# Kotstantinovskiy/SonicDiffusionBayesLab

Measured on AMD Instinct MI355X. Metric: 512x512 images/sec at 50 DDIM steps, higher is better.
Workload: dtype bf16; 1 GPU; SD-1.5 512x512 DDIM 50 steps, CFG 7.5, batch=8/GPU (BASELINE configs[1]); global_batch=8, sample_size=64, parallelism=batch-shard x1, weights=SD-1.5-shaped synthetic seed 1234

## Files before the change

### include/sd_hip.h

```cpp
#ifndef SD_HIP_H
#define SD_HIP_H

#ifdef __cplusplus
extern "C" {
#endif

typedef struct sd_unet sd_unet;

typedef struct sd_unet_config {
    int sample_size;
    int in_channels;
    int out_channels;
    int num_levels;
    int block_out_channels[8];
    int layers_per_block;
    int attn_levels[8];
    int cross_attention_dim;
    int num_heads;
    int norm_num_groups;
    float norm_eps;
    int context_len;
    int weight_dtype;
    float fp8_act_scale_norm;
    float fp8_act_scale_ff;
// ... 64 lines not shown
} sd_clip_config;
typedef struct sd_unet sd_clip;
int sd_clip_create(const sd_clip_config* cfg, sd_clip** out);
int sd_clip_encode(sd_clip* c, void* stream, const int* input_ids, int batch, float* hidden_out, void* workspace,
                   long long workspace_bytes);

typedef struct sd_clip_vision_config {
    int hidden_size;
    int num_layers;
    int num_heads;
    int intermediate_size;
    int image_size;
    int patch_size;
    int projection_dim;
    float layer_norm_eps;
} sd_clip_vision_config;
typedef struct sd_unet sd_clip_vision;
int sd_clip_create_projected(const sd_clip_config* cfg, int projection_dim, int eos_token_id, sd_clip** out);
long long sd_clip_text_embeds_workspace_bytes(sd_clip* c, int batch);
int sd_clip_text_embeds(sd_clip* c, void* stream, const int* input_ids, int batch, float* text_embeds, void* workspace,
                        long long workspace_bytes);
int sd_clip_vision_create(const sd_clip_vision_config* cfg, sd_clip_vision** out);
long long sd_clip_vision_workspace_bytes(sd_clip_vision* v, int batch, int height, int width);
int sd_clip_vision_encode(sd_clip_vision* v, void* stream, const unsigned char* images, int batch, int height, int width,
                          float* image_embeds, void* workspace, long long workspace_bytes);
int sd_clip_score(void* stream, const float* image_embeds, const float* text_embeds, int batch, int dim, float* raw,
                  float* score);
int sd_clip_resize_taps(int in_size, int out_size, int first, int count, int* xmin, int* xcnt, int* coeffs);

typedef struct sd_inception sd_inception;
int sd_inception_create(sd_inception** out);
void sd_inception_destroy(sd_inception* h);
int sd_inception_num_convs(const sd_inception* h);
int sd_inception_conv_info(const sd_inception* h, int index, char* name, int name_cap, long long shape[4]);
int sd_inception_load_conv(sd_inception* h, const char* name, const float* weight_oihw, long long weight_numel,
                           const float* bias, int cout);
int sd_inception_finalize(sd_inception* h);
long long sd_inception_workspace_bytes(sd_inception* h, int batch, int tap);
int sd_inception_features(sd_inception* h, void* stream, const unsigned char* images, int batch, int height, int width,
                          int tap, float* features, void* workspace, long long workspace_bytes);
int sd_fid_accumulate(void* stream, const float* features, int batch, int dim, double* sum, double* cov_sum,
                      long long* count);
int sd_op_inception_conv(void* stream, const void* X, const void* W, const float* bias, void* Y, int B, int Hin, int Win,
                         int Cin, int Cout, int kh, int kw, int stride, int pad_h, int pad_w, int ldy, int coff, int relu);
int sd_op_maxpool3x3(void* stream, const void* X, void* Y, int B, int H, int W, int C, int stride, int pad, int ldy, int coff);
int sd_op_avgpool3x3(void* stream, const void* X, void* Y, int B, int H, int W, int C, int ldy, int coff);
int sd_op_global_mean(void* stream, const void* X, float* out, int B, int HW, int C);
int sd_op_inception_resize(void* stream, const unsigned char* images, int B, int H, int W, void* out, int out_fp32);

#define SD_PROFILE_KINDS 32
int sd_unet_forward_profiled(sd_unet* u, void* stream, const float* latents, int latent_batch, int unet_batch,
                             float timestep, float* eps_out, void* workspace, long long workspace_bytes, int cache_mode,
                             int cache_branch_id, double kind_ms[SD_PROFILE_KINDS], long long kind_launches[SD_PROFILE_KINDS],
                             double kind_flops[SD_PROFILE_KINDS], double kind_bytes[SD_PROFILE_KINDS]);

long long sd_unet_forward_op_times(sd_unet* u, void* stream, const float* latents, int latent_batch, int unet_batch,
                                   float timestep, float* eps_out, void* workspace, long long workspace_bytes, int cache_mode,
                                   int cache_branch_id, char* text, long long cap);

int sd_unet_debug_tensor(sd_unet* u, void* stream, const char* name, float* host_out, long long numel,
                         void* workspace, int unet_batch, int cache_branch_id);

int sd_sched_step(void* stream, const float* eps, int cfg, float guidance, const float* x, const float* m1,
                  const float* m2, const float* m3, const float* noise, float* prev, float* y2, float* m_out,
                  const float coef[10], long long n);

int sd_cfg_rescale_factors(void* stream, const float* eps, int batch, long long n_per_sample, float guidance,
                           float rescale, float* k_out);
int sd_sched_step_rescaled(void* stream, const float* eps, int cfg, float guidance, const float* x, const float* m1,
                           const float* m2, const float* m3, const float* noise, float* prev, float* y2, float* m_out,
                           const float coef[10], long long n, const float* k, long long n_per_sample);

int sd_op_gemm(void* stream, const void* X, long long ldx, const void* X2, long long ldx2, int K1, const void* W,
               const float* bias, const float* bias2, const void* R, long long ldr, void* C, long long ldc, int M,
               int N, int K, int epi);
int sd_op_gemm_batched(void* stream, const void* X, long long ldx, const void* W, long long w_batch_stride,
                       int rows_per_batch, const float* bias, const void* R, long long ldr, void* C, long long ldc,
                       int M, int N, int K, int epi, int sm_valid);
int sd_op_gemm_batched_softmax_ln(void* stream, const void* X, long long ldx, const void* W, long long w_batch_stride,
                                  int rows_per_batch, void* C, long long ldc, int M, int N, int K, int sm_valid,
                                  const float* rowstats, int parts, const float* c1, const float* c2, float eps);
int sd_op_conv3x3(void* stream, const void* X, const void* W, const float* bias, const float* bias2, const void* R,
                  void* Y, int B, int Hin, int Win, int Cin, int Cout, int stride, int upsample);
int sd_op_conv3x3_down_asym(void* stream, const void* X, const void* W, const float* bias, void* Y, int B, int Hin, int Win,
                            int Cin, int Cout);
int sd_op_conv3x3_kernel(int M, int N, int Cin, int Hin, int Win, int stride, int upsample, int dtype);
int sd_op_softmax_rows(void* stream, void* S, long long rows, int cols, float scale);
int sd_op_conv3x3_upsample_subpixel(void* stream, const void* X, const void* W4, const float* bias, void* Y, int B, int Hin,
                                    int Win, int Cin, int Cout);
int sd_op_conv3x3_upsample_subpixel_groupnorm(void* stream, const void* X, const void* W4, const float* bias, void* Y, int B,
                                              int Hin, int Win, int Cin, int Cout, const float* gamma, const float* beta,
                                              void* Yn, int groups, float eps, int silu);
int sd_op_groupnorm(void* stream, const void* x1, int C1, const void* x2, int C2, const float* gamma,
                    const float* beta, void* y, int B, int HW, int groups, float eps, int silu);
int sd_op_conv3x3_groupnorm(void* stream, const void* X, const void* W, const float* bias, const float* bias2,
                            const void* R, void* Y, int B, int Hin, int Win, int Cin, int Cout, const float* gamma,
                            const float* beta, void* Yn, int groups, float eps, int silu);
int sd_op_conv3x3_splitk(int M, int Cout, int Cin, int Hin, int Win, int stride, int upsample);
int sd_op_layernorm(void* stream, const void* x, const float* gamma, const float* beta, void* y, int rows, int C,
                    float eps);
int sd_op_attention(void* stream, const void* Q, long long ldq, const void* K, long long ldk, const void* V,
                    long long ldv, void* O, long long ldo, int B, int heads, int Nq, int Nk, int D, float scale);
int sd_op_gemm_qkv_headmajor(void* stream, const void* X, long long ldx, const void* W, void* Q, void* KV, int M, int C,
                             int tokens, int K);
int sd_op_attention_headmajor(void* stream, const void* Q, long long ldq, const void* K, const void* V, void* O,
                              long long ldo, int B, int heads, int Nq, int Nk, int D, float scale);
int sd_op_clip_attention(void* stream, const void* qkv, void* out, int B, int L, int H, int heads);
int sd_op_vit_attention(void* stream, const void* qkv, void* out, int B, int L, int H, int heads);
int sd_op_clip_preprocess(void* stream, const unsigned char* images, int B, int H, int W, int S, int P, unsigned char* crop,
                          void* patches);
int sd_op_conv_in(void* stream, const float* x, int Bsrc, const float* Wt, const float* bias, void* y, int B, int H,
                  int W, int Cin, int Cout);
int sd_op_conv_out(void* stream, const void* x, const void* Wp, const float* bias, float* y, int B, int H, int W,
                   int Cin, int Cout);
int sd_op_time_embedding(void* stream, float t, const void* W1, const float* b1, const void* W2, const float* b2,
                         float* scratch, float* temb, int dim_in, int dim);
int sd_op_timestep_cond(void* stream, float t, const float* cond, const void* Wc, float* row, float* emb, int cond_dim,
                        int dim);

int sd_op_ln_partials(int kind, int M, int N);
int sd_op_gemm_rowstats(void* stream, const void* X, long long ldx, const void* W, const float* bias, const void* R,
                        long long ldr, void* C, long long ldc, int M, int N, int K, float* rowstats);
int sd_op_gemm_ln(void* stream, const void* X, long long ldx, const void* Wg, const float* c1, const float* c2,
                  const float* rowstats, int parts, float eps, void* C, long long ldc, int M, int N, int K, int epi);
int sd_op_gemm_plan(void* stream, const void* X, long long ldx, const void* X2, long long ldx2, int K1, const void* W,
                    const float* bias, const float* bias2, const void* R, long long ldr, void* C, long long ldc, int M, int N,
                    int K, float* rowstats, float* stats, const float* ln_rs, int ln_parts, const float* ln_c1, float ln_eps,
                    void* KV, int hm_tokens);
int sd_op_xattn_fused_rowstats(void* stream, const void* X, const void* R, void* Y, const void* At, const void* Bw,
                               const float* bias, int M, int C, int rows_per_sample, int L, float* rowstats);
int sd_op_xattn_fused(void* stream, const void* X, const void* R, void* Y, const void* At, const void* Bw,
                      const float* bias, int M, int C, int rows_per_sample, int L);
int sd_op_xattn_fused_ln(void* stream, const void* X, const void* R, void* Y, const void* At, const void* Bw,
                         const float* bias, int M, int C, int rows_per_sample, int L, const float* ln_rowstats, int ln_parts,
                         long long ln_rows, const float* c2, float eps, float* rowstats);
int sd_op_conv3x3_ablate(void* stream, const void* X, const void* W, void* Y, int B, int Hin, int Win, int Cin, int Cout,
                         int ablate);
int sd_op_xattn_fused_stamps(void* stream, const void* X, const void* R, void* Y, const void* At, const void* Bw,
                             const float* bias, int M, int C, int rows_per_sample, int L, unsigned long long* stamps);

int sd_op_gemm_fp8(void* stream, const void* X, long long ldx, const void* W, const float* wscale, float xscale,
                   const float* bias, const void* R, long long ldr, void* C, long long ldc, int M, int N, int K, int epi,
                   int out_fp8, float oscale);
int sd_op_conv3x3_fp8(void* stream, const void* X, const void* W, const float* wscale, float xscale, const float* bias,
                      const float* bias2, const void* R, void* Y, int B, int Hin, int Win, int Cin, int Cout, int stride,
                      int upsample);
int sd_op_groupnorm_fp8(void* stream, const void* x1, int C1, const void* x2, int C2, const float* gamma,
                        const float* beta, void* y, int B, int HW, int groups, float eps, int silu, int Cpad, float oscale);
int sd_op_layernorm_fp8(void* stream, const void* x, const float* gamma, const float* beta, void* y, int rows, int C,
                        int Cpad, float eps, float oscale);
int sd_op_quantize_fp8(void* stream, const void* x_bf16, void* y_fp8, long long rows, int C, int Cpad, float scale);

#ifdef __cplusplus
}
#endif
#endif
```

### sonicdiffusionbayeslab_amd/_lib.py

```python
from __future__ import annotations

import ctypes as C
import os
import re
from typing import Optional

HERE = os.path.dirname(os.path.abspath(__file__))
LIB_PATH = os.environ.get("SD_AMD_LIB", os.path.join(HERE, "lib", "libsdhip.so"))
HEADER_PATH = os.path.normpath(os.path.join(HERE, "..", "include", "sd_hip.h"))

ABLATE_LIB_PATH = os.path.join(HERE, "lib", "libsdhip_ablate.so")

_lib: Optional[C.CDLL] = None
_ablate: Optional[C.CDLL] = None


class SdUnetConfig(C.Structure):
    _fields_ = [
        ("sample_size", C.c_int), ("in_channels", C.c_int), ("out_channels", C.c_int),
        ("num_levels", C.c_int), ("block_out_channels", C.c_int * 8), ("layers_per_block", C.c_int),
        ("attn_levels", C.c_int * 8), ("cross_attention_dim", C.c_int), ("num_heads", C.c_int),
        ("norm_num_groups", C.c_int), ("norm_eps", C.c_float), ("context_len", C.c_int),
        ("weight_dtype", C.c_int), ("fp8_act_scale_norm", C.c_float), ("fp8_act_scale_ff", C.c_float),
        ("time_cond_proj_dim", C.c_int),
# ... 13 lines not shown

class SdClipVisionConfig(C.Structure):
    _fields_ = [
        ("hidden_size", C.c_int), ("num_layers", C.c_int), ("num_heads", C.c_int), ("intermediate_size", C.c_int),
        ("image_size", C.c_int), ("patch_size", C.c_int), ("projection_dim", C.c_int), ("layer_norm_eps", C.c_float),
    ]


class SdHipError(RuntimeError):
    pass


def declared_symbols() -> list:
    src = open(HEADER_PATH).read()
    src = re.sub(r"/\*.*?\*/", "", src, flags=re.S)
    return sorted(set(re.findall(r"\b(sd_[a-z0-9_]+)\s*\(", src)))


_vp, _i, _ll, _f = C.c_void_p, C.c_int, C.c_longlong, C.c_float
_SIGS = {
    "sd_last_error": (C.c_char_p, []),
    "sd_abi_version": (_i, []),
    "sd_unet_create": (_i, [C.POINTER(SdUnetConfig), C.POINTER(_vp)]),
    "sd_unet_destroy": (None, [_vp]),
    "sd_unet_num_params": (_i, [_vp]),
    "sd_unet_param_info": (_i, [_vp, _i, C.c_char_p, _i, C.POINTER(_ll), C.POINTER(_i)]),
    "sd_unet_load_param": (_i, [_vp, C.c_char_p, _vp, _ll]),
    "sd_unet_finalize": (_i, [_vp]),
    "sd_unet_debug_packed": (_ll, [_vp, C.c_char_p, _vp, _ll]),
    "sd_unet_calibrate_fp8": (_i, [_vp, _vp, _vp, _i, _i, _f, _f, _vp, _ll]),
    "sd_unet_fp8_scale_count": (_i, [_vp]),
    "sd_unet_fp8_scale_info": (_i, [_vp, _i, C.c_char_p, _i, C.POINTER(_f), C.POINTER(_f)]),
    "sd_unet_set_fp8_scale": (_i, [_vp, C.c_char_p, _f]),
    "sd_unet_workspace_bytes": (_ll, [_vp, _i, _i]),
    "sd_unet_set_context": (_i, [_vp, _vp, _vp, _i, _i, _vp, _ll]),
    "sd_unet_set_timestep_cond": (_i, [_vp, _vp, _vp]),
    "sd_unet_forward": (_i, [_vp, _vp, _vp, _i, _i, _f, _vp, _vp, _ll, _i, _i]),
    "sd_unet_workspace_bytes_hw": (_ll, [_vp, _i, _i, _i, _i]),
    "sd_unet_set_context_hw": (_i, [_vp, _vp, _vp, _i, _i, _i, _i, _vp, _ll]),
    "sd_unet_forward_hw": (_i, [_vp, _vp, _vp, _i, _i, _i, _i, _f, _vp, _vp, _ll, _i, _i]),
    "sd_unet_forward_profiled": (_i, [_vp, _vp, _vp, _i, _i, _f, _vp, _vp, _ll, _i, _i, C.POINTER(C.c_double),
                                      C.POINTER(_ll), C.POINTER(C.c_double), C.POINTER(C.c_double)]),
    "sd_unet_forward_op_times": (_ll, [_vp, _vp, _vp, _i, _i, _f, _vp, _vp, _ll, _i, _i, C.c_char_p, _ll]),
    "sd_vae_create": (_i, [C.POINTER(SdUnetConfig), C.POINTER(_vp)]),
    "sd_vae_decode": (_i, [_vp, _vp, _vp, _i, _f, _vp, _vp, _ll]),
    "sd_vae_decode_hw": (_i, [_vp, _vp, _vp, _i, _i, _i, _f, _vp, _vp, _ll]),
    "sd_vae_encoder_create": (_i, [C.POINTER(SdUnetConfig), C.POINTER(_vp)]),
    "sd_vae_encode_hw": (_i, [_vp, _vp, _vp, _i, _i, _i, _vp, _vp, _ll]),
    "sd_vae_posterior_sample": (_i, [_vp, _vp, _vp, _f, _vp, _i, _ll]),
    "sd_clip_create": (_i, [C.POINTER(SdClipConfig), C.POINTER(_vp)]),
    "sd_clip_encode": (_i, [_vp, _vp, _vp, _i, _vp, _vp, _ll]),
    "sd_clip_create_projected": (_i, [C.POINTER(SdClipConfig), _i, _i, C.POINTER(_vp)]),
    "sd_clip_text_embeds_workspace_bytes": (_ll, [_vp, _i]),
    "sd_clip_text_embeds": (_i, [_vp, _vp, _vp, _i, _vp, _vp, _ll]),
    "sd_clip_vision_create": (_i, [C.POINTER(SdClipVisionConfig), C.POINTER(_vp)]),
    "sd_clip_vision_workspace_bytes": (_ll, [_vp, _i, _i, _i]),
    "sd_clip_vision_encode": (_i, [_vp, _vp, _vp, _i, _i, _i, _vp, _vp, _ll]),
    "sd_clip_score": (_i, [_vp, _vp, _vp, _i, _i, _vp, _vp]),
    "sd_clip_resize_taps": (_i, [_i, _i, _i, _i, _vp, _vp, _vp]),
    "sd_op_vit_attention": (_i, [_vp, _vp, _vp, _i, _i, _i, _i]),
    "sd_op_clip_preprocess": (_i, [_vp, _vp, _i, _i, _i, _i, _i, _vp, _vp]),
    "sd_inception_create": (_i, [C.POINTER(_vp)]),
    "sd_inception_destroy": (None, [_vp]),
    "sd_inception_num_convs": (_i, [_vp]),
    "sd_inception_conv_info": (_i, [_vp, _i, C.c_char_p, _i, C.POINTER(_ll)]),
    "sd_inception_load_conv": (_i, [_vp, C.c_char_p, _vp, _ll, _vp, _i]),
    "sd_inception_finalize": (_i, [_vp]),
    "sd_inception_workspace_bytes": (_ll, [_vp, _i, _i]),
    "sd_inception_features": (_i, [_vp, _vp, _vp, _i, _i, _i, _i, _vp, _vp, _ll]),
    "sd_fid_accumulate": (_i, [_vp, _vp, _i, _i, _vp, _vp, _vp]),
    "sd_op_inception_conv": (_i, [_vp, _vp, _vp, _vp, _vp, _i, _i, _i, _i, _i, _i, _i, _i, _i, _i, _i, _i, _i]),
    "sd_op_maxpool3x3": (_i, [_vp, _vp, _vp, _i, _i, _i, _i, _i, _i, _i, _i]),
    "sd_op_avgpool3x3": (_i, [_vp, _vp, _vp, _i, _i, _i, _i, _i, _i]),
    "sd_op_global_mean": (_i, [_vp, _vp, _vp, _i, _i, _i]),
    "sd_op_inception_resize": (_i, [_vp, _vp, _i, _i, _i, _vp, _i]),
    "sd_unet_debug_tensor": (_i, [_vp, _vp, C.c_char_p, _vp, _ll, _vp, _i, _i]),
    "sd_sched_step": (_i, [_vp, _vp, _i, _f, _vp, _vp, _vp, _vp, _vp, _vp, _vp, _vp, C.POINTER(_f), _ll]),
    "sd_cfg_rescale_factors": (_i, [_vp, _vp, _i, _ll, _f, _f, _vp]),
    "sd_sched_step_rescaled": (_i, [_vp, _vp, _i, _f, _vp, _vp, _vp, _vp, _vp, _vp, _vp, _vp, C.POINTER(_f), _ll, _vp, _ll]),
    "sd_op_gemm": (_i, [_vp, _vp, _ll, _vp, _ll, _i, _vp, _vp, _vp, _vp, _ll, _vp, _ll, _i, _i, _i, _i]),
    "sd_op_gemm_batched": (_i, [_vp, _vp, _ll, _vp, _ll, _i, _vp, _vp, _ll, _vp, _ll, _i, _i, _i, _i, _i]),
    "sd_op_gemm_batched_softmax_ln": (_i, [_vp, _vp, _ll, _vp, _ll, _i, _vp, _ll, _i, _i, _i, _i, _vp, _i, _vp, _vp, _f]),
    "sd_op_conv3x3": (_i, [_vp, _vp, _vp, _vp, _vp, _vp, _vp, _i, _i, _i, _i, _i, _i, _i]),
    "sd_op_conv3x3_down_asym": (_i, [_vp, _vp, _vp, _vp, _vp, _i, _i, _i, _i, _i]),
    "sd_op_conv3x3_ablate": (_i, [_vp, _vp, _vp, _vp, _i, _i, _i, _i, _i, _i]),
    "sd_op_conv3x3_upsample_subpixel": (_i, [_vp, _vp, _vp, _vp, _vp, _i, _i, _i, _i, _i]),
    "sd_op_conv3x3_upsample_subpixel_groupnorm": (_i, [_vp, _vp, _vp, _vp, _vp, _i, _i, _i, _i, _i, _vp, _vp, _vp, _i, _f, _i]),
    "sd_op_groupnorm": (_i, [_vp, _vp, _i, _vp, _i, _vp, _vp, _vp, _i, _i, _i, _f, _i]),
    "sd_op_conv3x3_groupnorm": (_i, [_vp, _vp, _vp, _vp, _vp, _vp, _vp, _i, _i, _i, _i, _i, _vp, _vp, _vp, _i, _f, _i]),
    "sd_op_conv3x3_splitk": (_i, [_i, _i, _i, _i, _i, _i, _i]),
    "sd_op_conv3x3_kernel": (_i, [_i, _i, _i, _i, _i, _i, _i, _i]),
    "sd_op_softmax_rows": (_i, [_vp, _vp, _ll, _i, _f]),
    "sd_op_layernorm": (_i, [_vp, _vp, _vp, _vp, _vp, _i, _i, _f]),
    "sd_op_attention": (_i, [_vp, _vp, _ll, _vp, _ll, _vp, _ll, _vp, _ll, _i, _i, _i, _i, _i, _f]),
    "sd_op_gemm_qkv_headmajor": (_i, [_vp, _vp, _ll, _vp, _vp, _vp, _i, _i, _i, _i]),
    "sd_op_attention_headmajor": (_i, [_vp, _vp, _ll, _vp, _vp, _vp, _ll, _i, _i, _i, _i, _i, _f]),
    "sd_op_clip_attention": (_i, [_vp, _vp, _vp, _i, _i, _i, _i]),
    "sd_op_conv_in": (_i, [_vp, _vp, _i, _vp, _vp, _vp, _i, _i, _i, _i, _i]),
    "sd_op_conv_out": (_i, [_vp, _vp, _vp, _vp, _vp, _i, _i, _i, _i, _i]),
    "sd_op_time_embedding": (_i, [_vp, _f, _vp, _vp, _vp, _vp, _vp, _vp, _i, _i]),
    "sd_op_timestep_cond": (_i, [_vp, _f, _vp, _vp, _vp, _vp, _i, _i]),
    "sd_op_ln_partials": (_i, [_i, _i, _i]),
    "sd_op_gemm_rowstats": (_i, [_vp, _vp, _ll, _vp, _vp, _vp, _ll, _vp, _ll, _i, _i, _i, _vp]),
    "sd_op_gemm_plan": (_i, [_vp, _vp, _ll, _vp, _ll, _i, _vp, _vp, _vp, _vp, _ll, _vp, _ll, _i, _i, _i, _vp, _vp, _vp, _i, _vp, _f,
                            _vp, _i]),
    "sd_op_gemm_ln": (_i, [_vp, _vp, _ll, _vp, _vp, _vp, _vp, _i, _f, _vp, _ll, _i, _i, _i, _i]),
    "sd_op_xattn_fused_rowstats": (_i, [_vp, _vp, _vp, _vp, _vp, _vp, _vp, _i, _i, _i, _i, _vp]),
    "sd_op_xattn_fused": (_i, [_vp, _vp, _vp, _vp, _vp, _vp, _vp, _i, _i, _i, _i]),
    "sd_op_xattn_fused_ln": (_i, [_vp, _vp, _vp, _vp, _vp, _vp, _vp, _i, _i, _i, _i, _vp, _i, _ll, _vp, _f, _vp]),
    "sd_op_xattn_fused_stamps": (_i, [_vp, _vp, _vp, _vp, _vp, _vp, _vp, _i, _i, _i, _i, _vp]),
    "sd_op_gemm_fp8": (_i, [_vp, _vp, _ll, _vp, _vp, _f, _vp, _vp, _ll, _vp, _ll, _i, _i, _i, _i, _i, _f]),
    "sd_op_conv3x3_fp8": (_i, [_vp, _vp, _vp, _vp, _f, _vp, _vp, _vp, _vp, _i, _i, _i, _i, _i, _i, _i]),
    "sd_op_groupnorm_fp8": (_i, [_vp, _vp, _i, _vp, _i, _vp, _vp, _vp, _i, _i, _i, _f, _i, _i, _f]),
    "sd_op_layernorm_fp8": (_i, [_vp, _vp, _vp, _vp, _vp, _i, _i, _i, _f, _f]),
    "sd_op_quantize_fp8": (_i, [_vp, _vp, _vp, _ll, _i, _i, _f]),
}


def load() -> C.CDLL:
    global _lib
    if _lib is not None:
        return _lib
    if not os.path.exists(LIB_PATH):
        raise SdHipError(
            f"{LIB_PATH} is missing: build it with `python -m sonicdiffusionbayeslab_amd.build` "
            "(or __graft_entry__.build()).  There is no CPU/PyTorch fallback for the hot path.")
    lib = C.CDLL(LIB_PATH)
    for name, (res, args) in _SIGS.items():
        fn = getattr(lib, name)
        fn.restype = res
        fn.argtypes = args
    _lib = lib
    return lib


def load_ablate() -> C.CDLL:
    global _ablate
    if _ablate is not None:
        return _ablate
    if not os.path.exists(ABLATE_LIB_PATH):
        raise SdHipError(f"{ABLATE_LIB_PATH} is missing: build it with `python -m sonicdiffusionbayeslab_amd.build`")
    lib = C.CDLL(ABLATE_LIB_PATH)
    for name, (res, args) in _SIGS.items():
        fn = getattr(lib, name)
        fn.restype = res
        fn.argtypes = args
    _ablate = lib
    return lib


def check(rc: int, what: str = "libsdhip call", lib: Optional[C.CDLL] = None) -> None:
    if rc != 0:
        msg = (lib or load()).sd_last_error()
        raise SdHipError(f"{what} failed (rc={rc}): {msg.decode() if msg else '?'}")


def ptr(t) -> Optional[int]:
    return None if t is None else t.data_ptr()


def current_stream() -> int:
    import torch
    return torch.cuda.current_stream().cuda_stream
```

### sonicdiffusionbayeslab_amd/csrc/conv_halo.hip

```cpp
#include "common.h"
#include "kernels.h"

#include <stdlib.h>

#include <algorithm>

namespace {

constexpr int BM = 256, BN = 160;
constexpr int TN = 5, WTN = 80;
constexpr int HSLOTS = 400;
constexpr int HBYTES = HSLOTS * 128;
constexpr int WPIECES = BN / 8;
constexpr int WBYTES = WPIECES * 1024;
constexpr int WSTAGES = 3;
constexpr int SMEM = 2 * HBYTES + WSTAGES * WBYTES;
static_assert(SMEM <= 160 * 1024, "halo tile does not fit the 160 KiB LDS");
constexpr unsigned NOSRC = 0xffffffffu;

template <int N>
__device__ __forceinline__ void wait_vmcnt() {
    asm volatile("s_waitcnt vmcnt(%0)" ::"n"(N) : "memory");
}

__device__ __forceinline__ int swz_of(int row, int dt) { return dt ? (((row >> 1) & 1) | (row & 4)) : (row & 7); }

template <int DT, int DIAG = 0, int NWV = 8, int SUB = 0, int GEN = 0>
__global__ __launch_bounds__(NWV * 64, NWV == 8 ? 2 : 1) void conv_halo_kernel(const GemmArgs p) {
    static_assert(NWV == 8 || (NWV == 4 && DT == 0), "4-wave layout: bf16 only");
    static_assert(!SUB || (DT == 0 && DIAG == 0 && NWV == 8), "sub-pixel upsampler: bf16, 8 waves");
    static_assert(!GEN || (SUB == 0 && DIAG == 0 && NWV == 8), "geometry mode: 9 taps, 8 waves");
    constexpr int NTAP = SUB ? 4 : 9;
    constexpr int NT = NWV * 64;
    constexpr int WMW = NWV == 8 ? 4 : 2;
    constexpr int TM = BM / WMW / 16, WTM = TM * 16;
    constexpr int HPIECES = NWV == 8 ? 7 : 13;
    constexpr int WPW = NWV == 8 ? 3 : 5;
    constexpr bool CARRY = NWV == 4;
    constexpr int ESZ = DT ? 1 : 2;
    extern __shared__ __attribute__((aligned(16))) char smem[];
    const int tid = threadIdx.x, lane = tid & 63;
    const int wave = __builtin_amdgcn_readfirstlane(tid >> 6);

    int work = blockIdx.x;
    {
        const int nblk = gridDim.x;
        const int q = nblk >> 3, r = nblk & 7, xcd = work & 7, idx = work >> 3;
        work = (xcd < r ? xcd * (q + 1) : r * (q + 1) + (xcd - r) * q) + idx;
    }
    const int ntiles = p.tiles_m * p.tiles_n;
    const int nwork = ntiles * (SUB ? 4 : p.splitk);
    if (work >= nwork) return;
    const int S = (p.Cin * ESZ) >> 7;
    const int Mrows = SUB ? p.M >> 2 : p.M;

    const int up = SUB ? 0 : p.up;
    const int Ho = SUB ? p.Hin : p.Hout, Wo = SUB ? p.Win : p.Wout, HWo = Ho * Wo;
    const int RW = GEN ? p.rows_per_batch : min(Ho, BM / Wo);
    const int PW = p.Win + 2, PP = ((RW >> up) + 2) * PW;
    const int PIX = RW * Wo;
    const int HP = GEN ? PP : (BM / PIX) * PP;
    const int tpi = GEN ? (Ho + RW - 1) / RW : 1;

    const char* Xb = (const char*)p.X;
    const char* Wg = (const char*)p.W;

    constexpr int HREL_ZERO = (int)0x80000000;
    const int lgW = __builtin_ctz(Wo), lgHW = __builtin_ctz(HWo);
    const int RWin = RW >> up;
    int hrel[HPIECES];
    int hyv[GEN ? HPIECES : 1];
    const int jdup = wave < 2 ? HPIECES - 1 : HPIECES - 2;
#pragma unroll
    for (int j = 0; j < HPIECES; ++j) {
        const int L = (j == HPIECES - 1 ? jdup : j) * NT + tid;
        const int slot = L >> 3, cpos = L & 7;
        const int i = slot / PP, rem = slot - i * PP;
        const int hy = rem / PW, hx = rem - hy * PW;
        const bool ok = slot < HP && hx >= 1 && hx <= p.Win;
        hrel[j] = ok ? ((((hy - 1) * p.Win + (hx - 1)) * p.Cin * ESZ + ((cpos ^ swz_of(slot, DT)) << 4)) | i |
                        (hy == 0 ? 4 : 0) | (hy == RWin + 1 ? 8 : 0))
                     : HREL_ZERO;
        if (GEN) hyv[j] = hy;
    }

    auto wpiece = [&](int i) { return NWV == 4 ? wave + 4 * i : (i < 2 ? wave + 8 * i : (wave < 4 ? wave + 16 : wave + 8)); };

    int split = 0, m0 = 0, n0 = 0, s_begin = 0, s_end = 0, phase = 0;
    int mend = 0;
    unsigned hoff[HPIECES];
    unsigned woffs[WPW];
    auto setup = [&](int w) {
        int tile_n, tile_m;
        if (SUB) {
            const int C = 4 * p.tiles_n, rect = (p.tiles_m >> 3) * (C >> 2) * 32;
            const bool rects = gridDim.x == 256 && p.tune == 0;
            int combo;
            if (rects && w < rect) {
                const int r = w >> 5, i = w & 31, bc = r % (C >> 2);
                tile_m = (r / (C >> 2)) * 8 + (i >> 2);
                combo = bc * 4 + (i & 3);
            } else {
                const int w2 = rects ? w - rect : w;
                tile_m = (rects ? (p.tiles_m & ~7) : 0) + w2 / C;
                combo = w2 % C;
            }
            tile_n = combo % p.tiles_n;
            phase = combo / p.tiles_n;
            split = 0; s_begin = 0; s_end = S;
        } else {
            split = w / ntiles;
            const int t = w - split * ntiles;
// ... 8 lines not shown
            m0 = b * HWo + y0 * Wo;
            mend = m0 + min(RW, Ho - y0) * Wo;
            const int ybase = y0 >> up;
            const unsigned base = (unsigned)(((long)b * p.Hin + ybase) * p.Win * p.Cin * ESZ);
#pragma unroll
            for (int j = 0; j < HPIECES; ++j) {
                const int iy = ybase - 1 + hyv[j];
                const bool ok = hrel[j] != HREL_ZERO && iy >= 0 && iy < p.Hin;
                hoff[j] = ok ? base + (unsigned)(hrel[j] & ~15) : NOSRC;
            }
        } else {
#pragma unroll
        for (int j = 0; j < HPIECES; ++j) {
            const int mp = m0 + (hrel[j] & 3) * PIX;
            const int b = mp >> lgHW;
            const int ybase = (mp & (HWo - 1)) >> (lgW + up);
            const bool ok = hrel[j] != HREL_ZERO && mp < Mrows && !((hrel[j] & 4) && ybase == 0) &&
                            !((hrel[j] & 8) && ybase + RWin == p.Hin);
            const unsigned base = (unsigned)(((long)b * p.Hin + ybase) * p.Win * p.Cin * ESZ);
            hoff[j] = ok ? base + (unsigned)(hrel[j] & ~15) : NOSRC;
        }
        }
#pragma unroll
        for (int i = 0; i < WPW; ++i) {
            const int pc = wpiece(i);
            const int n = n0 + pc * 8 + (lane >> 3);
            const int c = (lane & 7) ^ swz_of(lane >> 3, DT);
            woffs[i] = n < p.N ? (unsigned)(((SUB ? (long)phase * p.w_batch_stride : 0l) + (long)n * p.ldw) * ESZ + (c << 4)) : NOSRC;
        }
    };
    const unsigned xbytes = (unsigned)((long)(Mrows / HWo) * p.Hin * p.Win * p.Cin * ESZ);
    const unsigned wbytes = (unsigned)((long)p.N * p.ldw * ESZ * (SUB ? 4 : 1));
    auto issue_h = [&](int j, int s, char* hb) {
        const __amdgpu_buffer_rsrc_t r = __builtin_amdgcn_make_buffer_rsrc((void*)Xb, 0, (int)(s >= 0 ? xbytes : 0u), 0x00020000);
        __builtin_amdgcn_raw_ptr_buffer_load_lds(r, LDS_PTR(hb + ((j == HPIECES - 1 ? jdup : j) * NWV + wave) * 1024), 16, (int)hoff[j],
                                                 s >= 0 ? s * 128 : 0, 0, 0);
    };
    auto issue_w1 = [&](int i, int kk, char* wb) {
        const __amdgpu_buffer_rsrc_t r = __builtin_amdgcn_make_buffer_rsrc((void*)Wg, 0, (int)(kk >= 0 ? wbytes : 0u), 0x00020000);
        __builtin_amdgcn_raw_ptr_buffer_load_lds(r, LDS_PTR(wb + wpiece(i) * 1024), 16, (int)woffs[i], kk >= 0 ? kk * 128 : 0, 0, 0);
    };
    auto issue_h_tap = [&](int tap, int s, char* hb) {
        if (SUB) {
            if (tap < 3) {
                issue_h(2 * tap, s, hb);
                issue_h(2 * tap + 1, s, hb);
            } else {
                issue_h(6, s, hb);
            }
        } else if (NWV == 8) {
            if (tap < 7) issue_h(tap, s, hb);
        } else if (tap < 5) {
            issue_h(2 * tap, s, hb);
            issue_h(2 * tap + 1, s, hb);
        } else if (tap < 8) {
            issue_h(tap + 5, s, hb);
        }
    };
    auto issue_w = [&](int kk, char* wb) {
#pragma unroll
        for (int i = 0; i < WPW; ++i) issue_w1(i, kk, wb);
    };

    const int wm = wave % WMW, wn = wave / WMW;
    const int lrow = lane & 15, lq = lane >> 4;
    int hbase[TM], hrc[TM];
#pragma unroll
    for (int f = 0; f < TM; ++f) {
        if (GEN) {
            const int pt = min(wm * WTM + f * 16 + lrow, PIX - 1);
            const int row = pt / Wo;
            hrc[f] = row << 16 | (pt - row * Wo);
            hbase[f] = PW + 1;
        } else {
        const int pt = wm * WTM + f * 16 + lrow;
        const int i = pt / PIX, rem = pt - i * PIX;
        hrc[f] = (rem >> lgW) << 16 | (rem & (Wo - 1));
        hbase[f] = i * PP + PW + 1;
        }
    }
    const int wfrag = (wn * WTN + lrow) * 128;
    const int wswz0 = DT ? ((2 * lq) ^ swz_of(lane, 1)) << 4 : (lq ^ (lane & 7)) << 4;

    auto frag_addr = [&](int f, int tp) -> int {
        const int hp = hbase[f] + (((hrc[f] >> 16) + (tp / 3 - 1)) >> up) * PW + (((hrc[f] & 0xffff) + (tp % 3 - 1)) >> up);
        return hp * 128 + (DT ? (((2 * lq) ^ swz_of(hp, 1)) << 4) : ((lq ^ (hp & 7)) << 4));
    };

    auto frag_addr_sub = [&](int f, int t) -> int {
        const int hp = hbase[f] + ((hrc[f] >> 16) + (phase >> 1) + (t >> 1) - 1) * PW + ((hrc[f] & 0xffff) + (phase & 1) + (t & 1) - 1);
        return hp * 128 + ((lq ^ (hp & 7)) << 4);
    };

    f32x4 acc[TN][TM];
    bf16x8 xf0[TM], wf0[TN], xf1[TM], wf1[TN];
    int xan[TM];
#pragma unroll
    for (int f = 0; f < TM; ++f) xan[f] = frag_addr(f, 0);
    auto mfmas = [&](const bf16x8* xf, const bf16x8* wf) {
#pragma unroll
        for (int a = 0; a < TN; ++a)
#pragma unroll
            for (int b = 0; b < TM; ++b)
                acc[a][b] = __builtin_amdgcn_mfma_f32_16x16x32_bf16(wf[a], xf[b], acc[a][b], 0, 0, 0);
    };
    i32x8 wq[DT ? TN : 1], xq[2];
    auto ld32 = [&](const char* base, int off) -> i32x8 {
        return cat_u32x4(*(const u32x4*)(base + off), *(const u32x4*)(base + (off ^ 16)));
    };

    char* const Hb0 = smem;
    char* const Hb1 = smem + HBYTES;
    char* const Wb = smem + 2 * HBYTES;

    int hsel = 0, wst = 0;
    setup(work);
#pragma unroll
    for (int j = 0; j < HPIECES; ++j) issue_h(j, s_begin, Hb0);
    issue_w(s_begin * NTAP, Wb);
    issue_w(s_begin * NTAP + 1, Wb + WBYTES);
    bool stores_pending = false;
    constexpr int FULL_STORES = (TN / 2 + TN % 2) * TM;

    while (true) {
#pragma unroll
        for (int a = 0; a < TN; ++a)
#pragma unroll
            for (int b = 0; b < TM; ++b) acc[a][b] = f32x4{0.f, 0.f, 0.f, 0.f};
        if (CARRY) {
#pragma unroll
            for (int f = 0; f < TM; ++f) xf1[f] = bf16x8{0, 0, 0, 0, 0, 0, 0, 0};
#pragma unroll
            for (int a = 0; a < TN; ++a) wf1[a] = bf16x8{0, 0, 0, 0, 0, 0, 0, 0};
        }

        for (int s = s_begin; s < s_end; ++s) {
            const char* hcur = hsel ? Hb1 : Hb0;
            char* hnext = hsel ? Hb0 : Hb1;
            const bool more = s + 1 < s_end;
            if (DT || NWV == 4) {
#pragma unroll
                for (int f = 0; f < TM; ++f) asm volatile("" : "+v"(hbase[f]), "+v"(hrc[f]));
            }
#pragma unroll
            for (int tap = 0; tap < NTAP; ++tap) {
                if (SUB) {
                    if (tap == 0) {
                        if (s == s_begin && stores_pending) wait_vmcnt<3 + FULL_STORES>();
                        else wait_vmcnt<3>();
                    } else {
                        wait_vmcnt<5>();
                    }
                } else if (DIAG == 0) {
                if (NWV == 8) {
                if (tap == 0) {
                    if (s == s_begin && stores_pending) wait_vmcnt<3 + FULL_STORES>();
                    else wait_vmcnt<3>();
                } else if (tap == 8) {
                    wait_vmcnt<3>();
                } else {
                    wait_vmcnt<4>();
                }
                } else {
                if (tap == 0) {
                    if (s == s_begin && stores_pending) wait_vmcnt<5 + FULL_STORES>();
                    else wait_vmcnt<5>();
// ... 20 lines not shown
                    }
                    if ((DIAG & 8) && tap == 0 && s == s_begin) {
#pragma unroll
                        for (int f = 0; f < TM; ++f) xf1[f] = xf0[f];
#pragma unroll
                        for (int a = 0; a < TN; ++a) wf1[a] = wf0[a];
                    }
                    __builtin_amdgcn_sched_barrier(0);
                    const int hs = more ? s + 1 : -1, kw = s * 9 + tap + 2 < s_end * 9 ? s * 9 + tap + 2 : -1;
#pragma unroll
                    for (int a = 0; a < TN; ++a) {
#pragma unroll
                        for (int b = 0; b < TM; ++b) {
                            acc[a][b] = __builtin_amdgcn_mfma_f32_16x16x32_bf16(wf1[a], xf1[b], acc[a][b], 0, 0, 0);
                            const int idx = a * TM + b;
                            if (idx % 5 == 4 && !(DIAG & 2)) {
                                const int pc = idx / 5;
                                if (pc < WPW) issue_w1(pc, kw, wnext);
                                else if (tap < 5 && pc < WPW + 2) issue_h(2 * tap + (pc - WPW), hs, hnext);
                                else if (tap < 8 && pc == WPW) issue_h(tap + 5, hs, hnext);
                            }
                        }
                    }
                    __builtin_amdgcn_sched_barrier(0);
                    if (!(DIAG & 8)) {
#pragma unroll
                    for (int f = 0; f < TM; ++f) xf1[f] = *(const bf16x8*)(hcur + (xa[f] ^ 64));
#pragma unroll
                    for (int a = 0; a < TN; ++a) wf1[a] = *(const bf16x8*)(wcur + wfrag + a * 2048 + (wswz0 ^ 64));
                    }
#pragma unroll
                    for (int f = 0; f < TM; ++f) xan[f] = frag_addr(f, tap == 8 ? 0 : tap + 1);
                    mfmas(xf0, wf0);
                    __builtin_amdgcn_sched_barrier(0);
                    __builtin_amdgcn_s_waitcnt(0xc07f);
                } else if (DT) {
#pragma unroll
                    for (int a = 0; a < TN; ++a) wq[a] = ld32(wcur, wfrag + a * 2048 + wswz0);
                    xq[0] = ld32(hcur, xa[0]);
                    __builtin_amdgcn_sched_barrier(0);
                    issue_h_tap(tap, more ? s + 1 : -1, hnext);
                    issue_w(s * 9 + tap + 2 < s_end * 9 ? s * 9 + tap + 2 : -1, wnext);
                    __builtin_amdgcn_sched_barrier(0);
#pragma unroll
                    for (int b = 0; b < TM; ++b) {
                        if (b + 1 < TM) xq[(b + 1) & 1] = ld32(hcur, xa[b + 1]);
#pragma unroll
                        for (int a = 0; a < TN; ++a)
                            acc[a][b] = __builtin_amdgcn_mfma_scale_f32_16x16x128_f8f6f4(wq[a], xq[b & 1], acc[a][b], 0, 0, 0, 0, 0, 0);
                    }
                } else {
                    if (!(DIAG & 8)) {
#pragma unroll
                    for (int f = 0; f < TM; ++f) xf0[f] = *(const bf16x8*)(hcur + xa[f]);
#pragma unroll
                    for (int a = 0; a < TN; ++a) wf0[a] = *(const bf16x8*)(wcur + wfrag + a * 2048 + wswz0);
                    }
                    __builtin_amdgcn_sched_barrier(0);
                    if (!(DIAG & 2)) {
                    issue_h_tap(tap, more ? s + 1 : -1, hnext);
                    issue_w(s * NTAP + tap + 2 < s_end * NTAP ? s * NTAP + tap + 2 : -1, wnext);
                    }
                    __builtin_amdgcn_sched_barrier(0);
                    if (!(DIAG & 8)) {
#pragma unroll
                    for (int f = 0; f < TM; ++f) xf1[f] = *(const bf16x8*)(hcur + (xa[f] ^ 64));
#pragma unroll
                    for (int a = 0; a < TN; ++a) wf1[a] = *(const bf16x8*)(wcur + wfrag + a * 2048 + (wswz0 ^ 64));
                    } else if (tap == 0 && s == s_begin) {
#pragma unroll
                        for (int f = 0; f < TM; ++f) xf0[f] = xf1[f] = *(const bf16x8*)(hcur + xa[f]);
#pragma unroll
                        for (int a = 0; a < TN; ++a) wf0[a] = wf1[a] = *(const bf16x8*)(wcur + wfrag + a * 2048 + wswz0);
                    }
                    mfmas(xf0, wf0);
                    mfmas(xf1, wf1);
                }
                wst = wst == 2 ? 0 : wst + 1;
            }
            hsel ^= 1;
        }
        if (CARRY) mfmas(xf1, wf1);

        const int em0 = m0, en0 = n0, esplit = split, ephase = phase;
        const int elim = GEN ? mend : Mrows;
        auto crow = [&](int m) -> long {
            if (!SUB) return m;
            const int b = m >> lgHW, ml = m & (HWo - 1);
            return ((long)b * p.Hout + 2 * (ml >> lgW) + (ephase >> 1)) * p.Wout + 2 * (ml & (Wo - 1)) + (ephase & 1);
        };
        if (DT && p.splitk == 1) {
#pragma unroll
            for (int a = 0; a < TN; ++a) {
                const int n = min(en0 + wn * WTN + a * 16 + lq * 4, p.N - 4);
                const f32x4 sv = *(const f32x4*)(p.wscale + n) * p.xscale_inv;
#pragma unroll
                for (int b = 0; b < TM; ++b) acc[a][b] *= sv;
            }
        }
        if (p.splitk == 1) {
            if (p.R) {
                u32x2 rr[TN][TM];
#pragma unroll
                for (int a = 0; a < TN; ++a) {
                    const int n = min(en0 + wn * WTN + a * 16 + lq * 4, p.N - 4);
#pragma unroll
                    for (int b = 0; b < TM; ++b) {
                        const int m = min(em0 + wm * WTM + b * 16 + lrow, elim - 1);
                        rr[a][b] = *(const u32x2*)(p.R + crow(m) * p.ldr + n);
                    }
                }
#pragma unroll
                for (int a = 0; a < TN; ++a)
#pragma unroll
                    for (int b = 0; b < TM; ++b) {
                        acc[a][b][0] += bflo(rr[a][b][0]); acc[a][b][1] += bfhi(rr[a][b][0]);
                        acc[a][b][2] += bflo(rr[a][b][1]); acc[a][b][3] += bfhi(rr[a][b][1]);
                    }
            }
            if (p.bias) {
#pragma unroll
                for (int a = 0; a < TN; ++a) {
                    const int n = min(en0 + wn * WTN + a * 16 + lq * 4, p.N - 4);
                    f32x4 bv = *(const f32x4*)(p.bias + n);
                    if (p.bias2) bv += *(const f32x4*)(p.bias2 + n);
#pragma unroll
                    for (int b = 0; b < TM; ++b) acc[a][b] += bv;
                }
            }
        }

        work += gridDim.x;
        const bool more_work = work < nwork;
        const bool wide_ok = (p.ldc & 7) == 0;
        if (more_work) {
            setup(work);
            wait_vmcnt<0>();
            char* hb = hsel ? Hb1 : Hb0;
#pragma unroll
            for (int j = 0; j < HPIECES; ++j) issue_h(j, s_begin, hb);
            issue_w(s_begin * NTAP, Wb + wst * WBYTES);
            issue_w(s_begin * NTAP + 1, Wb + (wst == 2 ? 0 : wst + 1) * WBYTES);
            stores_pending = p.splitk == 1 && wide_ok && (em0 + BM <= elim) && (en0 + BN <= p.N);
        }

        if (p.splitk > 1) {
            float* slab = p.slab + (long)esplit * p.M * p.N;
#pragma unroll
            for (int a = 0; a < TN; ++a) {
                const int n = en0 + wn * WTN + a * 16 + lq * 4;
                if (n >= p.N) continue;
#pragma unroll
                for (int b = 0; b < TM; ++b) {
                    const int m = em0 + wm * WTM + b * 16 + lrow;
                    if (m >= (GEN ? elim : p.M)) continue;
                    *(f32x4*)(slab + (long)m * p.N + n) = acc[a][b];
                }
            }
        } else {
            if (!GEN && p.stats) {
                const int r0 = em0 + wm * WTM;
                const int blk0 = SUB ? ((((r0 >> lgHW) << 2) + ephase) << (lgHW - 6)) + ((r0 & (HWo - 1)) >> 6) : r0 >> 6;
#pragma unroll
                for (int hb64 = 0; hb64 < TM / 4; ++hb64)
                    tile_channel_stats<TN, TM>(acc, p.stats, blk0 + hb64, p.N, en0 + wn * WTN, p.N,
                                               em0 + wm * WTM, Mrows, lane, 4 * hb64, 4);
            }
            auto store_narrow = [&](int a) {
                const int n = en0 + wn * WTN + a * 16 + lq * 4;
                if (n >= p.N) return;
#pragma unroll
                for (int b = 0; b < TM; ++b) {
                    const int m = em0 + wm * WTM + b * 16 + lrow;
                    const f32x4 v = acc[a][b];
                    u32x2 o = {pack2bf(v[0], v[1]), pack2bf(v[2], v[3])};
                    if (m < elim) *(u32x2*)(p.C + crow(m) * p.ldc + n) = o;
                }
            };
#pragma unroll
            for (int a = 0; a < TN; a += 2) {
                const int nb = en0 + wn * WTN + a * 16;
                if (a + 1 < TN && wide_ok && nb + 32 <= p.N) {
#pragma unroll
                    for (int b = 0; b < TM; ++b) {
                        const int m = em0 + wm * WTM + b * 16 + lrow;
                        const f32x4 vx = acc[a][b], vy = acc[a + 1 < TN ? a + 1 : a][b];
                        const auto s0 = __builtin_amdgcn_permlane16_swap(pack2bf(vx[0], vx[1]), pack2bf(vy[0], vy[1]), false, false);
                        const auto s1 = __builtin_amdgcn_permlane16_swap(pack2bf(vx[2], vx[3]), pack2bf(vy[2], vy[3]), false, false);
                        const u32x4 o = {s0[0], s1[0], s0[1], s1[1]};
                        const int col = nb + (lq & 1) * 16 + (lq >> 1) * 8;
                        if (m < elim) *(u32x4*)(p.C + crow(m) * p.ldc + col) = o;
                    }
                } else {
                    store_narrow(a);
                    if (a + 1 < TN) store_narrow(a + 1);
                }
            }
        }
        if (!more_work) break;
    }
}

bool halo_enabled() {
    static const char* env = getenv("SD_CONV_HALO");
    return env ? atoi(env) != 0 : true;
}

}

static bool pow2_applicable(const GemmArgs& a);
static int launch_halo_gen(GemmArgs a, hipStream_t stream);

bool sd_conv_halo_applicable(const GemmArgs& a) {
    return sd_conv_halo_mode(a) != 0;
}

static int gen_rows(const GemmArgs& a) {
    const int H = a.Hin << a.up, W = a.Win << a.up;
    if (W < 8 || W > BM) return 0;
    int rw = std::min(H, BM / W);
    if (a.up) rw &= ~1;
    while (rw > 0 && ((rw >> a.up) + 2) * (a.Win + 2) > HSLOTS) rw -= a.up ? 2 : 1;
    return rw;
}

int sd_conv_halo_mode(const GemmArgs& a) {
    if (!halo_enabled() || a.stride != 1) return 0;
    const long ldw0 = a.ldw ? a.ldw : a.K;
    if ((long)a.M * a.Cin * 2 >= (1l << 32) || (long)a.N * ldw0 * 2 >= (1l << 32)) return 0;
    if (a.dt == 1 && a.Cin % 128) return 0;
    if (pow2_applicable(a)) return 1;
    const char* env = getenv("SD_CONV_HALO_GEN");
    if ((env && atoi(env) == 0) || a.subpix || a.stats) return 0;
    const int H = a.Hin << a.up, W = a.Win << a.up;
    if (a.M % (H * W)) return 0;
    const int rw = gen_rows(a);
    return rw > 0 && rw * W >= 192 ? 2 : 0;
}

static bool pow2_applicable(const GemmArgs& a) {
    if (!halo_enabled() || a.stride != 1) return false;
    const int H = a.Hin << a.up, W = a.Win << a.up;
    if (W < 8 || W > BM || BM % W) return false;
    const int RW = H < BM / W ? H : BM / W;
    const int PIX = RW * W;
    if (BM % PIX || (H * W) % PIX || (a.up && (RW & 1))) return false;
    if ((W & (W - 1)) || ((H * W) & (H * W - 1))) return false;
    if ((BM / PIX) * ((RW >> a.up) + 2) * (a.Win + 2) > HSLOTS) return false;
    const long ldw = a.ldw ? a.ldw : a.K;
    if ((long)a.M * a.Cin * 2 >= (1l << 32) || (long)a.N * ldw * 2 >= (1l << 32)) return false;
    if (a.dt == 1 && a.Cin % 128) return false;
    return true;
}

bool sd_conv_halo_subpix_applicable(const GemmArgs& a) {
    const char* env = getenv("SD_SUBPIX_HALO");
    const bool off = env && atoi(env) == 0;
    if (off || !a.subpix || a.dt != 0 || a.R != nullptr || (a.splitk > 1 && a.slab) || (a.Hin * a.Win) % 64 != 0) return false;
    GemmArgs g = a;
    g.up = 0; g.stride = 1; g.M = a.M / 4;
    if (!sd_conv_halo_applicable(g)) return false;
    const long ldw = a.ldw ? a.ldw : a.K;
    if ((long)a.N * 4 * ldw * 2 >= (1l << 32)) return false;
    if (a.w_batch_stride != (long)a.N * ldw) return false;
    return (long)((g.M + BM - 1) / BM) * 4 * ((a.N + BN - 1) / BN) >= 256;
}

int sd_conv_halo_splitk(int M, int N, int Cin, int dt) {
    const int tiles = ((M + BM - 1) / BM) * ((N + BN - 1) / BN);
    if (tiles >= 192) return 1;
    const int S = Cin / (dt ? 128 : 64);
    int want = (256 + tiles - 1) / tiles;
    int maxs = tiles < 64 ? S / 2 : S / 4;
    int s = want < maxs ? want : maxs;
    if (s > 8) s = 8;
    return s < 1 ? 1 : s;
}

int sd_conv3x3_splitk(int M, int N, int Cin, int Hin, int Win, int stride, int up, int dt) {
    static const char* env = getenv("SD_SPLITK");
    GemmArgs a;
    a.M = M; a.N = N; a.Cin = Cin; a.K = 9 * Cin; a.ldw = a.K; a.Hin = Hin; a.Win = Win; a.stride = stride; a.up = up; a.dt = dt;
    if (!env && sd_conv_halo_applicable(a)) return sd_conv_halo_splitk(M, N, Cin, dt);
    return sd_gemm_splitk(M, N, dt ? 9 * Cin / 2 : 9 * Cin, 128);
}

int sd_launch_conv3x3_halo(const GemmArgs& a0, hipStream_t stream) {
    GemmArgs a = a0;
    a.tiles_m = ((a.subpix ? a.M / 4 : a.M) + BM - 1) / BM;
    a.tiles_n = (a.N + BN - 1) / BN;
    if (a.ldw == 0) a.ldw = a.K;
    if (a.slab == nullptr || a.splitk < 1) a.splitk = 1;
    SD_REQUIRE(!a.defer_reduce || a.splitk > 1, "conv3x3 halo: defer_reduce needs split-K (the consumer would read an unwritten slab)");
    if (a.subpix) {
        SD_REQUIRE(a.dt == 0 && a.splitk == 1 && a.R == nullptr && a.up == 0 && a.K == 4 * a.Cin && a.w_batch_stride > 0 &&
                       a.Hout == 2 * a.Hin && a.Wout == 2 * a.Win && a.M % (4 * a.Hin * a.Win) == 0 && a0.tune == 0,
                   "conv3x3 halo, sub-pixel upsampler: bf16, no split-K, no residual, K = 4 Cin");
        SD_REQUIRE(a.w_batch_stride == (long)a.N * a.ldw, "conv3x3 halo, sub-pixel upsampler: phase stride %ld != N * ldw = %ld",
                   a.w_batch_stride, (long)a.N * a.ldw);
        static bool sub_attr_set = false;
        if (!sub_attr_set) {
            SD_CHECK_HIP(hipFuncSetAttribute((const void*)conv_halo_kernel<0, 0, 8, 1>, hipFuncAttributeMaxDynamicSharedMemorySize, SMEM));
            sub_attr_set = true;
        }
        int g = a.tiles_m * a.tiles_n * 4;
        if (g > 256) g = 256;
        static const bool old_order = getenv("SD_SUBPIX_ORDER") && atoi(getenv("SD_SUBPIX_ORDER")) == 0;
        a.tune = old_order ? 1 : 0;
        hipLaunchKernelGGL((conv_halo_kernel<0, 0, 8, 1>), dim3(g), dim3(512), SMEM, stream, a);
        SD_CHECK_HIP(hipGetLastError());
        return 0;
    }
    const int slices = a.Cin / (a.dt ? 128 : 64);
    SD_REQUIRE(a.splitk <= slices, "conv3x3 halo: splitk %d exceeds the %d channel slices", a.splitk, slices);
    if (!pow2_applicable(a0)) return launch_halo_gen(a, stream);
    static bool attr_set = false;
    if (!attr_set) {
        SD_CHECK_HIP(hipFuncSetAttribute((const void*)conv_halo_kernel<0>, hipFuncAttributeMaxDynamicSharedMemorySize, SMEM));
        SD_CHECK_HIP(hipFuncSetAttribute((const void*)conv_halo_kernel<1>, hipFuncAttributeMaxDynamicSharedMemorySize, SMEM));
#ifdef SD_ABLATE
        SD_CHECK_HIP(hipFuncSetAttribute((const void*)conv_halo_kernel<0, 1>, hipFuncAttributeMaxDynamicSharedMemorySize, SMEM));
        SD_CHECK_HIP(hipFuncSetAttribute((const void*)conv_halo_kernel<0, 3>, hipFuncAttributeMaxDynamicSharedMemorySize, SMEM));
        SD_CHECK_HIP(hipFuncSetAttribute((const void*)conv_halo_kernel<0, 7>, hipFuncAttributeMaxDynamicSharedMemorySize, SMEM));
        SD_CHECK_HIP(hipFuncSetAttribute((const void*)conv_halo_kernel<0, 15>, hipFuncAttributeMaxDynamicSharedMemorySize, SMEM));
        SD_CHECK_HIP(hipFuncSetAttribute((const void*)conv_halo_kernel<0, 0, 4>, hipFuncAttributeMaxDynamicSharedMemorySize, SMEM));
        SD_CHECK_HIP(hipFuncSetAttribute((const void*)conv_halo_kernel<0, 15, 4>, hipFuncAttributeMaxDynamicSharedMemorySize, SMEM));
#endif
        attr_set = true;
    }
    int grid = a.tiles_m * a.tiles_n * a.splitk;
    if (grid > 256) grid = 256;
#ifdef SD_ABLATE
    const int tune = a0.tune;
    a.tune = tune;
    static const int env_waves = getenv("SD_CONV_WAVES") ? atoi(getenv("SD_CONV_WAVES")) : 8;
    const int waves = (tune & 256) ? 4 : env_waves;
    if (a.dt) hipLaunchKernelGGL(conv_halo_kernel<1>, dim3(grid), dim3(512), SMEM, stream, a);
    else if (waves == 4 && (tune & 15) == 8) hipLaunchKernelGGL((conv_halo_kernel<0, 15, 4>), dim3(grid), dim3(256), SMEM, stream, a);
    else if (waves == 4 && (tune & 15) == 0) hipLaunchKernelGGL((conv_halo_kernel<0, 0, 4>), dim3(grid), dim3(256), SMEM, stream, a);
    else if ((tune & 15) == 1) hipLaunchKernelGGL((conv_halo_kernel<0, 1>), dim3(grid), dim3(512), SMEM, stream, a);
    else if ((tune & 15) == 2) hipLaunchKernelGGL((conv_halo_kernel<0, 3>), dim3(grid), dim3(512), SMEM, stream, a);
    else if ((tune & 15) == 4) hipLaunchKernelGGL((conv_halo_kernel<0, 7>), dim3(grid), dim3(512), SMEM, stream, a);
    else if ((tune & 15) == 8) hipLaunchKernelGGL((conv_halo_kernel<0, 15>), dim3(grid), dim3(512), SMEM, stream, a);
    else hipLaunchKernelGGL(conv_halo_kernel<0>, dim3(grid), dim3(512), SMEM, stream, a);
#else
    SD_REQUIRE(a0.tune == 0, "conv3x3 (halo): this build carries no ablation kernels (load libsdhip_ablate.so)");
    a.tune = 0;
    if (a.dt) hipLaunchKernelGGL(conv_halo_kernel<1>, dim3(grid), dim3(512), SMEM, stream, a);
    else hipLaunchKernelGGL(conv_halo_kernel<0>, dim3(grid), dim3(512), SMEM, stream, a);
#endif
    if (a.splitk > 1 && !a.defer_reduce) sd_launch_splitk_reduce(a, stream);
    SD_CHECK_HIP(hipGetLastError());
    return 0;
}

static int launch_halo_gen(GemmArgs a, hipStream_t stream) {
    const int Ho = a.Hin << a.up, Wo = a.Win << a.up, rw = gen_rows(a);
    SD_REQUIRE(rw > 0 && a.Hout == Ho && a.Wout == Wo && a.M % (Ho * Wo) == 0 && !a.stats && a.tune == 0,
               "conv3x3 halo (geometry mode): shape %dx%d -> %dx%d not taken", a.Hin, a.Win, Ho, Wo);
    a.rows_per_batch = rw;
    a.tiles_m = (a.M / (Ho * Wo)) * ((Ho + rw - 1) / rw);
    static bool attr_set = false;
    if (!attr_set) {
        SD_CHECK_HIP(hipFuncSetAttribute((const void*)conv_halo_kernel<0, 0, 8, 0, 1>, hipFuncAttributeMaxDynamicSharedMemorySize, SMEM));
        SD_CHECK_HIP(hipFuncSetAttribute((const void*)conv_halo_kernel<1, 0, 8, 0, 1>, hipFuncAttributeMaxDynamicSharedMemorySize, SMEM));
        attr_set = true;
    }
    int grid = a.tiles_m * a.tiles_n * a.splitk;
    if (grid > 256) grid = 256;
    if (a.dt) hipLaunchKernelGGL((conv_halo_kernel<1, 0, 8, 0, 1>), dim3(grid), dim3(512), SMEM, stream, a);
    else hipLaunchKernelGGL((conv_halo_kernel<0, 0, 8, 0, 1>), dim3(grid), dim3(512), SMEM, stream, a);
    if (a.splitk > 1 && !a.defer_reduce) sd_launch_splitk_reduce(a, stream);
    SD_CHECK_HIP(hipGetLastError());
    return 0;
}
```

### sonicdiffusionbayeslab_amd/csrc/gemm_conv.hip

```cpp
#include "common.h"
#include "kernels.h"

#include <stdlib.h>

#ifdef SD_ABLATE
#define SD_TUNE(p) ((p).tune)
#else
#define SD_TUNE(p) 0
#endif

namespace {

constexpr int AMODE_GEMM = 0;
constexpr int AMODE_CONV = 1;
constexpr int EPI_STD = 0;
constexpr int EPI_GEGLU = 1;
constexpr int EPI_SOFTMAX = 2;

constexpr int kPersistentGrid = 512;

template <int N>
__device__ __forceinline__ void wait_vmcnt() {
    asm volatile("s_waitcnt vmcnt(%0)" ::"n"(N) : "memory");
}
// ... 674 lines not shown
}

int sd_launch_gemm(const GemmArgs& a, int epi, hipStream_t stream) {
    if (check_stats(a, epi) || check_ln(a, epi) || check_headmajor(a, epi)) return -1;
    if (a.dt == 1) {
        if (check_fp8(a, "gemm")) return -1;
        SD_REQUIRE(a.N % 4 == 0 && a.M > 0 && a.N > 0 && a.zero_page, "gemm fp8: bad problem");
        SD_REQUIRE(a.ldx % 16 == 0 && (a.ldw == 0 || a.ldw % 16 == 0), "gemm fp8: row strides must be multiples of 16 bytes");
        if (epi == EPI_GEGLU) {
            SD_REQUIRE(a.N % 32 == 0, "geglu gemm: N=%d must be a multiple of 32", a.N);
            SD_REQUIRE(!a.out_fp8 || (a.ldc % 4 == 0), "geglu gemm fp8 out: ldc=%ld must be a multiple of 4 bytes", a.ldc);
            if (a.N % 256 == 0) return launch<256, 256, 4, 2, 2, AMODE_GEMM, EPI_GEGLU, 1>(a, stream);
            return launch<128, 128, 2, 2, 2, AMODE_GEMM, EPI_GEGLU, 1>(a, stream);
        }
        SD_REQUIRE(epi == EPI_STD && !a.out_fp8, "gemm fp8: epilogue %d not built", epi);
        return launch<128, 160, 2, 2, 2, AMODE_GEMM, EPI_STD, 1>(a, stream);
    }
    SD_REQUIRE(!a.out_fp8, "gemm: fp8 output needs fp8 operands");
    SD_REQUIRE(a.K % 64 == 0 && a.K >= 64, "gemm: K=%d must be a positive multiple of 64", a.K);
    SD_REQUIRE(a.N % 4 == 0, "gemm: N=%d must be a multiple of 4", a.N);
    SD_REQUIRE(a.K1 % 64 == 0 && a.K1 <= a.K, "gemm: K1=%d must be a multiple of 64 and <= K", a.K1);
    SD_REQUIRE(a.K1 == a.K || a.X2 != nullptr, "gemm: second K segment needs X2");
    SD_REQUIRE(a.M > 0 && a.N > 0, "gemm: empty problem");
    SD_REQUIRE(a.zero_page != nullptr, "gemm: zero page missing");
    const char* lean_env = getenv("SD_GEMM_LEAN");
    const bool lean_off = lean_env && atoi(lean_env) == 0;
    if (epi == EPI_GEGLU) {
        SD_REQUIRE(a.N % 32 == 0, "geglu gemm: N=%d must be a multiple of 32", a.N);
        if (!lean_off && big_tile_mode() == 0 && sd_gemm_lean_applicable(a, 1)) return sd_launch_gemm_lean(a, 1, 256, stream);
        if (big_tile_ok(a.M, a.N, 128)) return launch<256, 128, 4, 2, 3, AMODE_GEMM, EPI_GEGLU>(a, stream);
        if (big_tile_mode() != 3 && a.N % 256 == 0) return launch<256, 256, 4, 2, 2, AMODE_GEMM, EPI_GEGLU>(a, stream);
        return launch<128, 128, 2, 2, 2, AMODE_GEMM, EPI_GEGLU>(a, stream);
    }
    SD_REQUIRE(a.rows_per_batch == 0 || a.rows_per_batch % 128 == 0,
               "gemm: rows_per_batch=%d must be a multiple of the 128-row tile", a.rows_per_batch);
    if (epi == EPI_SOFTMAX) {
        SD_REQUIRE(a.N % 80 == 0 && a.sm_valid > 0 && a.sm_valid <= 80 && a.R == nullptr && (a.bias == nullptr || a.ln_rs),
                   "softmax gemm: N=%d must be a multiple of 80, 0 < sm_valid=%d <= 80, no bias/residual", a.N, a.sm_valid);
        SD_REQUIRE(!a.ln_per_sample || (a.ln_rs && a.rows_per_batch > 0), "gemm: per-sample LayerNorm vectors need per-sample weights");
        return launch<128, 160, 2, 2, 2, AMODE_GEMM, EPI_SOFTMAX>(a, stream);
    }
    if (a.rows_per_batch) return launch<128, 160, 2, 2, 2, AMODE_GEMM, EPI_STD>(a, stream);
    if (!lean_off && big_tile_mode() == 0 && sd_gemm_lean_applicable(a, epi)) {
        const int rows = (!a.stats && !a.ln_rs && !a.hm_C) ? sd_gemm_tile_rows(a.M, a.N, a.K) : 128;
        return sd_launch_gemm_lean(a, 0, rows, stream);
    }
    if (big_tile_ok(a.M, a.N, 160)) return launch<256, 160, 4, 2, 3, AMODE_GEMM, EPI_STD>(a, stream);
    if (big_tile_mode() == 2) return launch<256, 160, 4, 2, 2, AMODE_GEMM, EPI_STD>(a, stream);
    if (!a.stats && !a.ln_rs && sd_gemm_tile_rows(a.M, a.N, a.K) == 64) return launch<64, 160, 2, 2, 2, AMODE_GEMM, EPI_STD>(a, stream);
    return launch<128, 160, 2, 2, 2, AMODE_GEMM, EPI_STD>(a, stream);
}

int sd_launch_conv3x3(const GemmArgs& a, hipStream_t stream) {
    if (check_stats(a, EPI_STD)) return -1;
    if (a.dt == 1) {
        if (check_fp8(a, "conv3x3")) return -1;
        SD_REQUIRE(a.Cin % 128 == 0, "conv3x3 fp8: Cin=%d must be a multiple of 128 (pad the channels)", a.Cin);
    }
    SD_REQUIRE(a.Cin % 64 == 0, "conv3x3: Cin=%d must be a multiple of 64", a.Cin);
    if (a.subpix) {
        SD_REQUIRE(a.dt == 0 && a.K == 4 * a.Cin && a.N % 4 == 0 && a.Hout == 2 * a.Hin && a.Wout == 2 * a.Win && a.stride == 1 &&
                       a.up == 0 && (a.Hin * a.Win) % 64 == 0 && a.M % (4 * a.Hin * a.Win) == 0 && a.R == nullptr &&
                       a.zero_page != nullptr && a.w_batch_stride > 0 && !(a.splitk > 1 && a.slab),
                   "conv3x3 sub-pixel upsample: bf16, K = 4 Cin, low-res pixels per sample %% 64 == 0, no residual, no split-K");
        if (sd_conv_halo_subpix_applicable(a)) return sd_launch_conv3x3_halo(a, stream);
        if ((a.Hin * a.Win) % 128 != 0) {
            SD_REQUIRE(!a.stats, "conv3x3 sub-pixel upsample: block statistics need low-res pixels per sample %% 128 == 0");
            return launch<64, 160, 2, 2, 2, AMODE_CONV, EPI_STD>(a, stream);
        }
        return launch<128, 160, 2, 2, 2, AMODE_CONV, EPI_STD>(a, stream);
    }
    SD_REQUIRE(a.K == 9 * a.Cin, "conv3x3: K must be 9*Cin");
    SD_REQUIRE(a.N % 4 == 0, "conv3x3: Cout=%d must be a multiple of 4", a.N);
    SD_REQUIRE(a.stride == 1 || a.stride == 2, "conv3x3: stride %d", a.stride);
    SD_REQUIRE(!(a.up && a.stride != 1), "conv3x3: upsample needs stride 1");
    SD_REQUIRE(a.zero_page != nullptr, "conv3x3: zero page missing");
    const int hv = a.Hin << a.up, wv = a.Win << a.up;
    SD_REQUIRE(!a.asym || (a.stride == 2 && a.dt == 0 && a.Hin % 2 == 0 && a.Win % 2 == 0 && !a.stats),
               "conv3x3: the asymmetric form is bf16, stride 2, even input sides (%dx%d stride %d)", a.Hin, a.Win, a.stride);
    SD_REQUIRE(a.Hout == (hv + 2 - 3) / a.stride + 1 && a.Wout == (wv + 2 - 3) / a.stride + 1,
               "conv3x3: output size %dx%d inconsistent with input %dx%d stride %d up %d", a.Hout, a.Wout,
               a.Hin, a.Win, a.stride, a.up);
    SD_REQUIRE(a.M % (a.Hout * a.Wout) == 0, "conv3x3: M not a multiple of Hout*Wout");
    if (sd_conv_halo_applicable(a)) return sd_launch_conv3x3_halo(a, stream);
    if (a.dt == 1) return launch<128, 160, 2, 2, 2, AMODE_CONV, EPI_STD, 1>(a, stream);
    if (big_tile_ok(a.M, a.N, 160)) return launch<256, 160, 4, 2, 3, AMODE_CONV, EPI_STD>(a, stream);
    return launch<128, 160, 2, 2, 2, AMODE_CONV, EPI_STD>(a, stream);
}
```

### sonicdiffusionbayeslab_amd/csrc/kernels.h

```cpp
#pragma once
#include <vector>

#include "common.h"

struct GemmArgs {
    const bf16_t* X = nullptr;
    long ldx = 0;
    const bf16_t* X2 = nullptr;
    long ldx2 = 0;
    int K1 = 0;
    const bf16_t* W = nullptr;
    long ldw = 0;
    const float* bias = nullptr;
    const float* bias2 = nullptr;
    const bf16_t* R = nullptr;
    long ldr = 0;
    bf16_t* C = nullptr;
    long ldc = 0;
    int M = 0, N = 0, K = 0;
    int Hin = 0, Win = 0, Cin = 0, Hout = 0, Wout = 0, stride = 1, up = 0;
    int asym = 0;
    int splitk = 1;
    float* slab = nullptr;
    int defer_reduce = 0;
    const void* zero_page = nullptr;
    long w_batch_stride = 0;
    int rows_per_batch = 0;
    int sm_valid = 0;
    int tiles_m = 0, tiles_n = 0;
    int tune = 0;
    float* stats = nullptr;
    float* rowstats = nullptr;
    bf16_t* KV = nullptr;
    int hm_C = 0, hm_tok = 0;
    int subpix = 0;
    const float* ln_rs = nullptr;
    const float* ln_c1 = nullptr;
    int ln_np = 0;
    float ln_eps = 1e-5f;
    int ln_per_sample = 0;
    int dt = 0;
    const float* wscale = nullptr;
    float xscale_inv = 1.0f;
    int out_fp8 = 0;
    float oscale = 1.0f;
};

int sd_gemm_tile_rows(int M, int N, int K = 0);
int sd_gemm_splitk(int M, int N, int K, int rows = 0);
int sd_launch_gemm(const GemmArgs& a, int epi , hipStream_t stream);
int sd_launch_conv3x3(const GemmArgs& a, hipStream_t stream);
bool sd_gemm_lean_applicable(const GemmArgs& a, int epi);
int sd_launch_gemm_lean(const GemmArgs& a, int epi, int rows, hipStream_t stream);
void sd_launch_splitk_reduce(const GemmArgs& a, hipStream_t stream);
bool sd_conv_halo_applicable(const GemmArgs& a);
int sd_conv_halo_mode(const GemmArgs& a);
int sd_conv3x3_splitk(int M, int N, int Cin, int Hin, int Win, int stride, int up, int dt = 0);
bool sd_conv_halo_subpix_applicable(const GemmArgs& a);
int sd_launch_conv3x3_halo(const GemmArgs& a, hipStream_t stream);

struct GroupNormArgs {
    const bf16_t* x1 = nullptr; int C1 = 0;
    const bf16_t* x2 = nullptr; int C2 = 0;
    const float* gamma = nullptr; const float* beta = nullptr;
    bf16_t* y = nullptr;
    int out_fp8 = 0, Cpad = 0;
    float oscale = 1.0f;
    const float* stats1 = nullptr; const float* stats2 = nullptr;
    const float* slab = nullptr; int splitk = 0;
    const float* sbias = nullptr; const float* sbias2 = nullptr;
    const bf16_t* sR = nullptr; long sldr = 0;
    bf16_t* x1w = nullptr;
    float* partial = nullptr;
    int B = 0, HW = 0, groups = 32, nsplit = 0;
    float eps = 1e-5f;
    int silu = 0;
};
int sd_groupnorm_nsplit(int B, int HW);
bool sd_groupnorm_uses_small(int B, int HW, int C1, int C2, int groups);
bool sd_groupnorm_slab_ok(int B, int HW, int C1, int C2, int groups);
size_t sd_groupnorm_scratch_bytes(int B, int HW, int groups);
int sd_launch_groupnorm(const GroupNormArgs& a, hipStream_t stream);

int sd_launch_softmax_rows(bf16_t* s, long rows, int cols, float scale, hipStream_t stream);
int sd_launch_softmax_rows_long(bf16_t* s, long rows, int cols, float scale, hipStream_t stream);
int sd_launch_pqconv(const float* x, const float* W, const float* bias, float* y, int B, int HW, float in_scale,
                     hipStream_t stream);

int sd_launch_layernorm(const bf16_t* x, const float* gamma, const float* beta, bf16_t* y, int rows, int C,
                        float eps, hipStream_t stream);
int sd_launch_layernorm_fp8(const bf16_t* x, const float* gamma, const float* beta, void* y, int rows, int C, int Cpad,
                            float eps, float oscale, hipStream_t stream);
int sd_launch_amax_e4m3(const void* y, long nbytes, unsigned* out, hipStream_t stream);
int sd_launch_quantize_fp8(const bf16_t* x, void* y, long rows, int C, int Cpad, float scale, hipStream_t stream);

struct AttnArgs {
    const bf16_t* Q = nullptr; long ldq = 0;
    const bf16_t* K = nullptr; long ldk = 0;
    const bf16_t* V = nullptr; long ldv = 0;
    bf16_t* O = nullptr; long ldo = 0;
    int B = 0, heads = 0, Nq = 0, Nk = 0, D = 0;
    float scale = 0.f;
    const void* consts = nullptr;
    int kv_head_major = 0;
    int q_prescaled = 0;
    int xcd_order = 1;
};
int sd_launch_attention(const AttnArgs& a, hipStream_t stream);

int sd_launch_gemv(const float* x, const bf16_t* W, const float* b, float* y, int N, int K, int silu_in,
                   hipStream_t stream);
int sd_launch_timestep_sinusoid(float t, float* out, int dim, hipStream_t stream);
int sd_launch_timestep_sinusoid_row(float t, const float* row, float* out, int dim, hipStream_t stream);
int sd_launch_f32_to_bf16(const float* src, bf16_t* dst, long n, hipStream_t stream);
int sd_launch_transpose_bf16(const bf16_t* src, bf16_t* dst, int B, int R, int Cc, hipStream_t stream, int perm16 = 0);

int sd_launch_retile32(const bf16_t* src, bf16_t* dst, int B, int R, int K, int RT, hipStream_t stream);
int sd_launch_replicate(const void* src, void* dst, long bytes, int rep, hipStream_t stream);

struct XattnArgs {
    const bf16_t* X = nullptr;
    const bf16_t* R = nullptr;
    bf16_t* Y = nullptr;
    const bf16_t* At = nullptr;
    const bf16_t* Bw = nullptr;
    const float* bias = nullptr;
    int M = 0, C = 0, rows_per_sample = 0, L = 0;
    float* rowstats = nullptr;
    const float* ln_rs = nullptr; int ln_np = 0; long ln_rows = 0;
    const float* ln_c2 = nullptr;
    float ln_eps = 1e-5f;
    unsigned long long* stamps = nullptr;
};
bool sd_xattn_fused_applicable(int rows_per_sample, int C, int heads, int L);
int sd_xattn_slices(int M, int C);
int sd_launch_xattn_fused(const XattnArgs& a, hipStream_t stream);
int sd_launch_xattn_expand(const bf16_t* kv, bf16_t* out, int B, int L, int C, int NH, int col_off, float scale,
                           hipStream_t stream);
int sd_launch_clip_embed(const int* ids, const bf16_t* tok, const bf16_t* pos, bf16_t* out, int rows, int L, int H,
                         int vocab, hipStream_t stream);
int sd_launch_clip_attention(const bf16_t* qkv, bf16_t* out, int B, int L, int H, int heads, hipStream_t stream);
int sd_launch_quick_gelu(bf16_t* x, long n, hipStream_t stream);
// ... 50 lines not shown
```

### sonicdiffusionbayeslab_amd/csrc/unet.hip

```cpp
#include "../../include/sd_hip.h"
#include "common.h"
#include "kernels.h"

#include <stdarg.h>
#include <stdio.h>
#include <stdlib.h>
#include <string.h>
#include <sys/mman.h>

#include <algorithm>
#include <chrono>
#include <map>
#include <new>
#include <string>
#include <thread>
#include <tuple>
#include <unordered_map>
#include <vector>

static thread_local char g_err[1024] = "";
void sd_set_error(const char* fmt, ...) {
    va_list ap;
    va_start(ap, fmt);
    vsnprintf(g_err, sizeof(g_err), fmt, ap);
// ... 6 lines not shown
static void* g_scratch = nullptr;
static size_t g_scratch_bytes = 0;
static void* op_scratch(size_t bytes) {
    if (bytes > g_scratch_bytes) {
        (void)hipDeviceSynchronize();
        if (g_scratch) (void)hipFree(g_scratch);
        g_scratch = nullptr;
        g_scratch_bytes = 0;
        if (hipMalloc(&g_scratch, bytes) != hipSuccess) return nullptr;
        g_scratch_bytes = bytes;
    }
    return g_scratch;
}
static int ensure_zero_page() {
    if (g_zero_page) return 0;
    SD_CHECK_HIP(hipMalloc(&g_zero_page, 4096));
    SD_CHECK_HIP(hipMemset(g_zero_page, 0, 4096));
    const unsigned short one_chunk[8] = {0x3F80, 0, 0, 0, 0, 0, 0, 0};
    SD_CHECK_HIP(hipMemcpy((char*)g_zero_page + 256, one_chunk, sizeof(one_chunk), hipMemcpyHostToDevice));
    return 0;
}

namespace {

constexpr size_t NOFF = (size_t)-1;
constexpr int T_LATENTS = -2, T_EPS = -3;

struct ParamSpec {
    std::string name;
    std::vector<long long> shape;
    std::vector<float> data;
    bool loaded = false;
    long long numel() const {
        long long n = 1;
        for (auto s : shape) n *= s;
        return n;
    }
};

struct Wrap {
    int type;
    int block_i, layer_i;
};

enum OpKind { OP_SINUSOID, OP_GEMV, OP_CONV_IN, OP_GN, OP_CONV3, OP_GEMM, OP_LN, OP_ATTN, OP_CONV_OUT, OP_SOFTMAX, OP_PQCONV,
              OP_CLIP_EMBED, OP_CLIP_ATTN, OP_QGELU, OP_TO_F32, OP_XATTN, OP_REPLICATE,
              OP_VIT_PREP, OP_VIT_EMBED, OP_VIT_ATTN, OP_POOL, OP_CONV_IN_IMG, OP_ENC_OUT };

constexpr int REP_TEXT_POOLED = 2;

struct Op {
    int kind = 0;
    int x1 = -1, x2 = -1, r = -1, out = -1, aux = -1, b2t = -1;
    size_t w = NOFF, b = NOFF, g = NOFF, be = NOFF;
    long b2idx = 0;
    int M = 0, N = 0, K = 0, K1 = 0, epi = 0;
    int B = 0, Hin = 0, Win = 0, Cin = 0, Hout = 0, Wout = 0, stride = 1, up = 0;
    int C1 = 0, C2 = 0, HW = 0, silu = 0, nsplit = 0;
    float eps = 0.f;
    int heads = 0, D = 0, Nq = 0, Nk = 0;
    long ldq = 0, ldk = 0, ldv = 0, ldo = 0, qoff = 0, koff = 0, voff = 0;
    int silu_in = 0, splitk = 1;
    int pool_by_ids = 0;
    int defer = 0, slab_t = -1, slab_k = 0, slab_r = -1, slab_b2t = -1;
    size_t slab_b = NOFF;
    long slab_b2idx = 0;
    int wt = -1;
    size_t wx = NOFF;
    long xoff = 0, woff_el = 0, coff = 0, ldx_o = 0, ldw_o = 0, ldc_o = 0;
    float scale = 0.f;
    long wbs = 0;
    int rpb = 0, sm_valid = 0;
    int dt = 0, out_fp8 = 0, Cpad = 0, Kalg = 0;
    int sname = -1;
    int stats = -1, s1 = -1, s2 = -1;
    int subpix = 0;
    int asym = 0;
    int hm = 0;
    int qps = 0;
    int rs = -1, lnrs = -1, lnnp = 0;
    size_t c1 = NOFF;
    size_t wsc = NOFF;
    float xs = 1.f, os = 1.f;
    int nwrap = 0;
    Wrap wraps[3];
};

struct HostBlob {
    unsigned char* p = nullptr;
    size_t n = 0, cap = 0;
    unsigned char* data() { return p; }
    const unsigned char* data() const { return p; }
    size_t size() const { return n; }
    bool empty() const { return n == 0; }
    bool reserve(size_t bytes) {
        if (bytes <= cap) return true;
        void* q = mmap(nullptr, bytes, PROT_READ | PROT_WRITE, MAP_PRIVATE | MAP_ANONYMOUS | MAP_POPULATE, -1, 0);
        if (q == MAP_FAILED) return false;
        (void)madvise(q, bytes, MADV_HUGEPAGE);
        if (p) { memcpy(q, p, n); munmap(p, cap); }
        p = (unsigned char*)q; cap = bytes;
        return true;
    }
    void resize(size_t bytes) {
        if (bytes > cap && !reserve(std::max(bytes, cap * 2))) throw std::bad_alloc();
        n = bytes;
    }
    void release() { if (p) munmap(p, cap); p = nullptr; n = cap = 0; }
    ~HostBlob() { release(); }
    HostBlob() = default;
    HostBlob(const HostBlob&) = delete;
    HostBlob& operator=(const HostBlob&) = delete;
};

struct Tn {
    size_t bytes = 0;
    int def = -1, last = -1;
    bool persistent = false;
    bool ctx = false;
    size_t off = NOFF;
};

struct Plan {
    int UB = 0, branch = -1;
    int rep = 1;
    int lh = 0, lw = 0;
    std::vector<Tn> tensors;
    std::vector<Op> ops;
    std::vector<char> skipped;
    std::vector<int> ctx_kv;
    std::vector<size_t> ctx_w;
    std::vector<int> ctx_c;
    int ctx_bf16 = -1;
    struct Fold { int kv, at, bw, C; size_t wqT, wo; bool perm; int c2 = -1; size_t lnu = NOFF; int c1 = -1; size_t ones = NOFF; };
    std::vector<Fold> ctx_fold;
    int ctx_fold_scratch = -1;
    std::map<std::string, int> taps;
    size_t total_bytes = 0;
    ClipPrepGeom geom;
    std::vector<int> prep_tab;
    const int* dtab = nullptr;
};

}

struct sd_unet {
    int kind = 0;
    sd_unet_config cfg;
    sd_clip_config clip;
    sd_clip_vision_config vis;
    int text_proj = 0;
    int eos_id = -1;
    std::map<std::pair<int, int>, int*> prep_tabs;
    std::vector<ParamSpec> params;
    std::unordered_map<std::string, int> pindex;
    std::unordered_map<std::string, size_t> woff;
    HostBlob hblob;
    char* dweights = nullptr;
    bool finalized = false;
    bool debug_taps = false;
    bool fp8 = false;
    float s_norm = 8.f, s_ff = 2.f;
    std::vector<std::string> act_names;
    std::unordered_map<std::string, int> act_index;
    std::vector<float> act_scale, act_amax;
    int act_id(const std::string& name, float dflt) {
// ... 452 lines not shown
                s2 += (double)wv * beta[k];
            }
            c1[n] = (float)s1;
            c2[n] = (float)s2;
        }
    }
    void ff_out_merge(const std::string& p, const std::string& t, int C) {
        const auto& w2 = P(t + "ff.net.2.weight");
        const auto& b2 = P(t + "ff.net.2.bias");
        const auto& wpo = P(p + "proj_out.weight");
        const auto& bpo = P(p + "proj_out.bias");
        const int K4 = 4 * C, KT = 5 * C;
        std::vector<float> prod((size_t)C * K4, 0.f);
        const int nthreads = pack_threads();
        const bool avx2 = __builtin_cpu_supports("avx2") && __builtin_cpu_supports("fma");
        auto work = [&](int tid) {
            constexpr int NB = 8;
            for (int n0 = tid * NB; n0 + NB <= C; n0 += nthreads * NB) {
                float* dst[NB];
                float a[NB];
                for (int i = 0; i < NB; ++i) dst[i] = &prod[(size_t)(n0 + i) * K4];
                for (int c = 0; c < C; ++c) {
                    for (int i = 0; i < NB; ++i) a[i] = wpo[(size_t)(n0 + i) * C + c];
                    if (avx2) axpy_rows_avx2<NB>(dst, a, &w2[(size_t)c * K4], K4);
                    else axpy_rows_base<NB>(dst, a, &w2[(size_t)c * K4], K4);
                }
            }
        };
        std::vector<std::thread> th;
        for (int i = 1; i < nthreads; ++i) th.emplace_back(work, i);
        work(0);
        for (auto& x : th) x.join();
        const size_t woff = alloc(p + "ff_out.weight", (size_t)C * KT * 2);
        const size_t boff = alloc(p + "ff_out.bias", (size_t)C * 4);
        unsigned short* o = (unsigned short*)(u->hblob.data() + woff);
        float* bo = (float*)(u->hblob.data() + boff);
        for (int n = 0; n < C; ++n) {
            for (int k = 0; k < K4; ++k) o[(size_t)n * KT + k] = f32_to_bf16_host(prod[(size_t)n * K4 + k]);
            for (int c = 0; c < C; ++c) o[(size_t)n * KT + K4 + c] = f32_to_bf16_host(wpo[(size_t)n * C + c]);
            double acc = bpo[n];
            for (int c = 0; c < C; ++c) acc += (double)wpo[(size_t)n * C + c] * b2[c];
            bo[n] = (float)acc;
        }
    }
    void geglu(const std::string& t, int C) {
        const auto& w = P(t + "ff.net.0.proj.weight");
        const auto& b = P(t + "ff.net.0.proj.bias");
        const int H = 4 * C;
        size_t boff = alloc(t + "ff.geglu.bias", b.size() * 4);
        float* bo = (float*)(u->hblob.data() + boff);
        std::vector<float> perm(u->fp8 ? w.size() : 0);
        unsigned short* o = nullptr;
        if (!u->fp8) {
            const size_t woff = alloc(t + "ff.geglu.weight", w.size() * 2);
            o = (unsigned short*)(u->hblob.data() + woff);
        }
        for (int r = 0; r < 2 * H; ++r) {
            const int grp = r / 32, within = r % 32;
            const int src = within < 16 ? grp * 16 + within : H + grp * 16 + (within - 16);
            if (u->fp8) memcpy(&perm[(size_t)r * C], &w[(size_t)src * C], (size_t)C * 4);
            else for (int k = 0; k < C; ++k) o[(size_t)r * C + k] = f32_to_bf16_host(w[(size_t)src * C + k]);
            ((float*)(u->hblob.data() + boff))[r] = b[src];
        }
        (void)bo;
        if (u->fp8) quant_rows(t + "ff.geglu.weight", perm.data(), 2 * H, C, (C + 127) / 128 * 128);
        else {
            std::vector<float> pw((size_t)2 * H * C), pb(2 * H);
            for (int r = 0; r < 2 * H; ++r) {
                const int grp = r / 32, within = r % 32;
                const int src = within < 16 ? grp * 16 + within : H + grp * 16 + (within - 16);
                memcpy(&pw[(size_t)r * C], &w[(size_t)src * C], (size_t)C * 4);
                pb[r] = b[src];
            }
            ln_fold(t + "ff.geglu.weight", pw.data(), 2 * H, C, P(t + "norm3.weight"), P(t + "norm3.bias"), pb.data());
        }
    }
    void resnet(const std::string& p, int cin, int cout) {
        f32(p + "norm1.weight"); f32(p + "norm1.bias");
        f32(p + "conv1.bias");
        f32(p + "norm2.weight"); f32(p + "norm2.bias");
        f32(p + "conv2.bias");
        if (u->fp8) { conv3_fp8(p + "conv1.weight", cout, cin); conv3_fp8(p + "conv2.weight", cout, cout); }
        else { conv3(p + "conv1.weight", cout, cin); conv3(p + "conv2.weight", cout, cout); }
        if (cin != cout) { bf16_same(p + "conv_shortcut.weight"); f32(p + "conv_shortcut.bias"); }
    }
    void transformer(const std::string& p, int c) {
        f32(p + "norm.weight"); f32(p + "norm.bias");
        f32(p + "proj_in.bias");
        const std::string t = p + "transformer_blocks.0.";
        for (int i = 1; i <= 3; ++i) { f32(t + "norm" + std::to_string(i) + ".weight"); f32(t + "norm" + std::to_string(i) + ".bias"); }
        const float qs = 1.4426950408889634f / sqrtf((float)(c / u->cfg.num_heads));
        if (u->fp8) {
            fp8_same(p + "proj_in.weight", c, c);
            fp8_concat_rows(t + "attn1.qkv.weight", {t + "attn1.to_q.weight", t + "attn1.to_k.weight", t + "attn1.to_v.weight"}, c, qs);
            fp8_same(t + "ff.net.2.weight", c, 4 * c);
        } else {
            bf16_same(p + "proj_in.weight");
            concat_rows(t + "attn1.qkv.weight", {t + "attn1.to_q.weight", t + "attn1.to_k.weight", t + "attn1.to_v.weight"}, qs);
            {
                std::vector<float> all;
                for (const char* n : {"attn1.to_q.weight", "attn1.to_k.weight", "attn1.to_v.weight"})
                    all.insert(all.end(), P(t + n).begin(), P(t + n).end());
                for (size_t i = 0; i < (size_t)c * c; ++i) all[i] *= qs;
                ln_fold(t + "attn1.qkv.weight", all.data(), 3 * c, c, P(t + "norm1.weight"), P(t + "norm1.bias"), nullptr);
            }
            bf16_same(t + "ff.net.2.weight");
        }
        bf16_same(t + "attn1.to_out.0.weight"); f32(t + "attn1.to_out.0.bias");
        bf16_same(t + "attn2.to_q.weight");
        {
            const auto& d = P(t + "attn2.to_q.weight");
            size_t off = alloc(t + "attn2.to_q.weight.T", d.size() * 2);
            unsigned short* o = (unsigned short*)(u->hblob.data() + off);
            for (int r = 0; r < c; ++r)
                for (int k = 0; k < c; ++k) o[(size_t)r * c + k] = f32_to_bf16_host(d[(size_t)k * c + r]);
        }
        if (!u->fp8) {
            const auto& d = P(t + "attn2.to_q.weight");
            const auto& gm = P(t + "norm2.weight");
            const auto& bt = P(t + "norm2.bias");
            size_t off = alloc(t + "attn2.to_q.weight.T.ln", d.size() * 2);
            size_t uoff = alloc(t + "attn2.to_q.lnu", (size_t)c * 4);
            size_t ooff = alloc(t + "attn2.to_q.ones", (size_t)c * 4);
            for (int j = 0; j < c; ++j) ((float*)(u->hblob.data() + ooff))[j] = 1.0f;
            unsigned short* o = (unsigned short*)(u->hblob.data() + off);
            float* uu = (float*)(u->hblob.data() + uoff);
            for (int j = 0; j < c; ++j) {
                double m = 0.0, ub = 0.0;
                for (int cc = 0; cc < c; ++cc) {
                    m += (double)d[(size_t)j * c + cc] * gm[cc];
                    ub += (double)d[(size_t)j * c + cc] * bt[cc];
                }
                m /= c;
                uu[j] = (float)ub;
                for (int cc = 0; cc < c; ++cc) o[(size_t)cc * c + j] = f32_to_bf16_host((float)((double)d[(size_t)j * c + cc] * gm[cc] - m));
            }
        }
        if (!u->fp8)
            ln_fold(t + "attn2.to_q.weight", P(t + "attn2.to_q.weight").data(), c, c, P(t + "norm2.weight"), P(t + "norm2.bias"), nullptr);
        concat_rows(t + "attn2.kv.weight", {t + "attn2.to_k.weight", t + "attn2.to_v.weight"});
        bf16_same(t + "attn2.to_out.0.weight"); f32(t + "attn2.to_out.0.bias");
        geglu(t, c);
        f32(t + "ff.net.2.bias");
        bf16_same(p + "proj_out.weight"); f32(p + "proj_out.bias");
        if (!u->fp8) ff_out_merge(p, t, c);
    }
};

template <class FR, class FT>
void walk_blocks(const sd_unet_config& c, FR&& on_resnet, FT&& on_transformer) {
    const int nl = c.num_levels;
    int ch = c.block_out_channels[0];
    std::vector<int> skip_ch{ch};
    for (int i = 0; i < nl; ++i) {
        const int co = c.block_out_channels[i];
        const std::string bp = "down_blocks." + std::to_string(i) + ".";
        for (int j = 0; j < c.layers_per_block; ++j) {
            on_resnet(bp + "resnets." + std::to_string(j) + ".", ch, co);
            ch = co;
            if (c.attn_levels[i]) on_transformer(bp + "attentions." + std::to_string(j) + ".", co);
            skip_ch.push_back(co);
        }
        if (i < nl - 1) skip_ch.push_back(co);
    }
    on_resnet("mid_block.resnets.0.", ch, ch);
    on_transformer("mid_block.attentions.0.", ch);
    on_resnet("mid_block.resnets.1.", ch, ch);
// ... 273 lines not shown
        return pl.ops.back();
    }
    static int pad128(int c) { return (c + 127) / 128 * 128; }
    int gn(int x1, int c1, int x2, int c2, int hw, const std::string& g, const std::string& b, float eps, int silu,
           bool fq = false) {
        Op o; o.kind = OP_GN; o.x1 = x1; o.C1 = c1; o.x2 = x2; o.C2 = c2; o.HW = hw; o.B = UB;
        o.g = W(g); o.be = W(b); o.eps = eps; o.silu = silu;
        o.nsplit = sd_groupnorm_nsplit(UB, hw);
        o.aux = tensor(sd_groupnorm_scratch_bytes(UB, hw, u->cfg.norm_num_groups));
        if (hw % 64 == 0 && !sd_groupnorm_uses_small(UB, hw, c1, c2, u->cfg.norm_num_groups) && stats_of.count(x1) &&
            (x2 < 0 || stats_of.count(x2))) {
            o.s1 = stats_of[x1];
            o.s2 = x2 >= 0 ? stats_of[x2] : -1;
        }
        if (fq) {
            o.out_fp8 = 1; o.Cpad = pad128(c1 + c2); o.sname = u->act_id(stem(g), u->s_norm); o.os = u->act_scale[o.sname];
            o.out = tensor((size_t)UB * hw * o.Cpad); tscale[o.out] = o.os;
        } else o.out = tensor((size_t)UB * hw * (c1 + c2) * 2);
        push(o);
        return o.out;
    }
    int conv3(int x, int hin, int win, int cin, int cout, int stride, int up, const std::string& w, const std::string& b,
              long b2idx, int b2t, int r, bool fq = false) {
        Op o; o.kind = OP_CONV3; o.x1 = x; o.B = UB; o.Hin = hin; o.Win = win; o.Cin = cin; o.N = cout;
        o.stride = stride; o.up = up;
        o.Hout = ((hin << up) + 2 - 3) / stride + 1;
        o.Wout = ((win << up) + 2 - 3) / stride + 1;
        o.M = UB * o.Hout * o.Wout; o.K = 9 * cin; o.Kalg = o.K;
        o.b = W(b); o.b2t = b2t; o.b2idx = b2idx; o.r = r;
        if (fq) { o.dt = 1; o.Cin = pad128(cin); o.K = 9 * o.Cin; o.w = W(w + ".fp8"); o.wsc = W(w + ".scale"); o.xs = xscale(x); }
        else o.w = W(w);
        static const bool subpix_off = getenv("SD_CONV_SUBPIXEL") && atoi(getenv("SD_CONV_SUBPIXEL")) == 0;
        if (up && !fq && !subpix_off && u->kind == 0 && stride == 1 && r < 0 && b2t < 0 && (hin * win) % 64 == 0 &&
            u->woff.count(w + ".sub")) {
            o.subpix = 1; o.K = 4 * cin; o.Kalg = 4 * cin;
            o.w = W(w + ".sub"); o.splitk = 1;
            o.out = tensor((size_t)o.M * cout * 2);
            if ((hin * win) % 128 == 0) want_stats(o, o.M, cout);
            push(o);
            return o.out;
        }
        o.splitk = sd_conv3x3_splitk(o.M, o.N, o.Cin, hin, win, stride, up, o.dt);
        if (o.splitk > 1) o.aux = tensor((size_t)o.splitk * o.M * o.N * 4);
        o.out = tensor((size_t)o.M * cout * 2);
        GemmArgs g;
        g.M = o.M; g.N = o.N; g.Cin = o.Cin; g.K = o.K; g.ldw = o.K; g.Hin = hin; g.Win = win; g.Hout = o.Hout; g.Wout = o.Wout;
        g.stride = stride; g.up = up; g.dt = o.dt;
        if (sd_conv_halo_mode(g) != 2) want_stats(o, o.M, cout);
        push(o);
        return o.out;
    }
    int gemm(int x1, int k1, int x2, int k2, int M, int N, const std::string& w, const std::string& b, int r, int epi,
             bool fq = false, const std::string& oname = "") {
        Op o; o.kind = OP_GEMM; o.x1 = x1; o.x2 = x2; o.K1 = k1; o.K = k1 + k2; o.Kalg = o.K; o.M = M; o.N = N; o.epi = epi;
        o.b = b.empty() ? NOFF : W(b); o.r = r;
        if (fq) { o.dt = 1; o.K = o.K1 = pad128(k1); o.w = W(w + ".fp8"); o.wsc = W(w + ".scale"); o.xs = xscale(x1); }
        else o.w = W(w);
        o.splitk = epi ? 1 : sd_gemm_splitk(M, N, o.dt ? o.K / 2 : o.K, o.dt ? 128 : 0);
        if (o.splitk > 1) o.aux = tensor((size_t)o.splitk * M * N * 4);
        if (!oname.empty()) {
            o.out_fp8 = 1; o.sname = u->act_id(oname, u->s_ff); o.os = u->act_scale[o.sname]; o.Cpad = pad128(N / 2);
            o.out = tensor((size_t)M * o.Cpad); tscale[o.out] = o.os;
        } else o.out = tensor((size_t)M * (epi ? N / 2 : N) * 2);
        push(o);
        return o.out;
    }
    int ln(int x, int M, int C, const std::string& g, const std::string& b, bool fq = false) {
        Op o; o.kind = OP_LN; o.x1 = x; o.M = M; o.N = C; o.g = W(g); o.be = W(b); o.eps = 1e-5f;
        if (fq) {
            o.out_fp8 = 1; o.Cpad = pad128(C); o.sname = u->act_id(stem(g), u->s_norm); o.os = u->act_scale[o.sname];
            o.out = tensor((size_t)M * o.Cpad); tscale[o.out] = o.os;
        } else o.out = tensor((size_t)M * C * 2);
        push(o);
        return o.out;
    }
    int attn(int q, long qoff, long ldq, int kv, long koff, long voff, long ldkv, int nq, int nk, int C) {
        Op o; o.kind = OP_ATTN; o.x1 = q; o.x2 = kv; o.qoff = qoff; o.koff = koff; o.voff = voff;
        o.ldq = ldq; o.ldk = o.ldv = ldkv; o.ldo = C; o.B = UB; o.heads = u->cfg.num_heads; o.D = C / u->cfg.num_heads;
        o.Nq = nq; o.Nk = nk;
        o.out = tensor((size_t)UB * nq * C * 2);
        push(o);
        return o.out;
    }
    int resnet(const std::string& p, int x1, int c1, int x2, int c2, int cout, int rh, int rw, int tproj_t) {
        const int hw = rh * rw, cin = c1 + c2, M = UB * hw;
        const bool fq = u->fp8;
        int t1 = gn(x1, c1, x2, c2, hw, p + "norm1.weight", p + "norm1.bias", u->cfg.norm_eps, 1, fq);
        int t2 = conv3(t1, rh, rw, cin, cout, 1, 0, p + "conv1.weight", p + "conv1.bias", u->tproj_off.at(p), tproj_t, -1, fq);
        int t3 = gn(t2, cout, -1, 0, hw, p + "norm2.weight", p + "norm2.bias", u->cfg.norm_eps, 1, fq);
        int sc = x1;
        if (cin != cout) sc = gemm(x1, c1, x2, c2, M, cout, p + "conv_shortcut.weight", p + "conv_shortcut.bias", -1, 0);
        return conv3(t3, rh, rw, cout, cout, 1, 0, p + "conv2.weight", p + "conv2.bias", 0, -1, sc, fq);
    }
    int n_transformers = 0;
    int transformer(const std::string& p, int x, int C, int rh, int rw) {
        const int hw = rh * rw, L = u->cfg.context_len;
        int M = UB * hw;
        const std::string t = p + "transformer_blocks.0.";
        const bool fq = u->fp8;
        int g = gn(x, C, -1, 0, hw, p + "norm.weight", p + "norm.bias", 1e-6f, 0, fq);
        int h0 = gemm(g, C, -1, 0, M, C, p + "proj_in.weight", p + "proj_in.bias", -1, 0, fq);
        int qkv, rs = -1, np = 0;
        if (!fq && (np = want_rowstats(pl.ops.back(), M, C, rs)) > 0) {
            qkv = gemm_ln(h0, rs, np, M, 3 * C, C, t + "attn1.qkv.weight", 0);
        } else {
            int n1 = ln(h0, M, C, t + "norm1.weight", t + "norm1.bias", fq);
            qkv = gemm(n1, C, -1, 0, M, 3 * C, t + "attn1.qkv.weight", "", -1, 0, fq);
        }
        static const bool hm_off = (getenv("SD_ATTN_HEADMAJOR") && atoi(getenv("SD_ATTN_HEADMAJOR")) == 0) ||
                                   getenv("SD_ATTN_NO_PIPE") || getenv("SD_ATTN_NO_DMA") || getenv("SD_GEMM_BIG");
        const bool hm = !hm_off && C / u->cfg.num_heads == 40 && C % 160 == 0 && hw % 128 == 0 && hw >= 256 &&
                        sd_gemm_tile_rows(M, 3 * C) == 128 && pl.ops.back().splitk == 1;
        int a1;
        if (hm) {
            pl.ops.back().hm = 1;
            pl.ops.back().HW = hw;
            a1 = attn(qkv, 0, C, qkv, (long)M * C, 2l * M * C, C, hw, hw, C);
            pl.ops.back().hm = 1;
        } else {
            a1 = attn(qkv, 0, 3 * C, qkv, C, 2 * C, 3 * C, hw, hw, C);
        }
        pl.ops.back().qps = 1;
        int h1 = gemm(a1, C, -1, 0, M, C, t + "attn1.to_out.0.weight", t + "attn1.to_out.0.bias", h0, 0);
        const int to_out_op = (int)pl.ops.size() - 1;
        if (prefix_rep > 1) {
            x = replicate(x, (size_t)M * C * 2, prefix_rep);
            h1 = replicate(h1, (size_t)M * C * 2, prefix_rep);
            UB *= prefix_rep;
            M = UB * hw;
            prefix_rep = 1;
        }
        static const int fused_min_hw = getenv("SD_XATTN_FUSED") ? atoi(getenv("SD_XATTN_FUSED")) : 1024;
        static const int fold_max_hw = getenv("SD_XATTN_FOLD") ? atoi(getenv("SD_XATTN_FOLD")) : 1024;
        static const bool xln_off = getenv("SD_XATTN_LN") && atoi(getenv("SD_XATTN_LN")) == 0;
        const int NH = u->cfg.num_heads, NP = NH * 80;
        const int xmode = (fused_min_hw > 0 && hw >= fused_min_hw && sd_xattn_fused_applicable(hw, C, NH, L)) ? 0
                          : (hw <= fold_max_hw && hw % 128 == 0 && L <= 80) ? 1 : 2;
        int rs2 = -1, np2 = 0;
        const long rs2_rows = (long)pl.ops[to_out_op].M;
        const bool first_tf = n_transformers++ == 0;
        if (!fq && !xln_off && (xmode == 0 || (!first_tf && rs2_rows == M)) &&
            u->woff.count(t + (xmode == 2 ? "attn2.to_q.weight.ln" : "attn2.to_q.weight.T.ln"))) {
            if (first_tf) pl.ops[to_out_op].splitk = 1;
            np2 = want_rowstats(pl.ops[to_out_op], (int)rs2_rows, C, rs2);
        }
        int n2 = np2 > 0 ? h1 : ln(h1, M, C, t + "norm2.weight", t + "norm2.bias");
        int kv = ctx_tensor((size_t)UB * L * 2 * C * 2);
        pl.ctx_kv.push_back(kv);
        pl.ctx_w.push_back(W(t + "attn2.kv.weight"));
        pl.ctx_c.push_back(C);
        int h2;
        if (xmode == 0) {
            int at = ctx_tensor((size_t)UB * NP * C * 2), bw = ctx_tensor((size_t)UB * C * NP * 2);
            Plan::Fold fd{kv, at, bw, C, W(t + (np2 > 0 ? "attn2.to_q.weight.T.ln" : "attn2.to_q.weight.T")), W(t + "attn2.to_out.0.weight"), true};
            if (np2 > 0) { fd.c2 = ctx_tensor((size_t)UB * NP * 4); fd.lnu = W(t + "attn2.to_q.lnu"); }
            pl.ctx_fold.push_back(fd);
            Op o; o.kind = OP_XATTN; o.x1 = n2; o.r = h1; o.wt = at; o.x2 = bw; o.M = M; o.N = C; o.K = NP; o.rpb = hw;
            o.sm_valid = L; o.b = W(t + "attn2.to_out.0.bias"); o.heads = NH;
            if (np2 > 0) { o.lnrs = rs2; o.lnnp = np2; o.s1 = fd.c2; o.ldx_o = rs2_rows; }
            o.out = tensor((size_t)M * C * 2); push(o); h2 = o.out;
        } else if (xmode == 1) {
            int at = ctx_tensor((size_t)UB * NP * C * 2), bw = ctx_tensor((size_t)UB * C * NP * 2);
            Plan::Fold fd{kv, at, bw, C, W(t + (np2 > 0 ? "attn2.to_q.weight.T.ln" : "attn2.to_q.weight.T")), W(t + "attn2.to_out.0.weight"), false};
            if (np2 > 0) {
                fd.c2 = ctx_tensor((size_t)UB * NP * 4); fd.lnu = W(t + "attn2.to_q.lnu");
                fd.c1 = ctx_tensor((size_t)UB * NP * 4); fd.ones = W(t + "attn2.to_q.ones");
            }
            pl.ctx_fold.push_back(fd);
            int pr;
            { Op o; o.kind = OP_GEMM; o.x1 = n2; o.K1 = C; o.K = C; o.M = M; o.N = NP; o.epi = 2; o.sm_valid = L;
              o.wt = at; o.wbs = (long)NP * C; o.rpb = hw;
              if (np2 > 0) { o.lnrs = rs2; o.lnnp = np2; o.s1 = fd.c1; o.s2 = fd.c2; }
              o.out = tensor((size_t)M * NP * 2); push(o); pr = o.out; }
            { Op o; o.kind = OP_GEMM; o.x1 = pr; o.K1 = NP; o.K = NP; o.M = M; o.N = C; o.epi = 0;
// ... 214 lines not shown
        pl.ctx_fold_scratch = ctx_tensor((size_t)3 * UB * c.num_heads * 80 * c.block_out_channels[nl - 1] * 2);
        int t_sin = tensor((size_t)c0 * 4), t_h1 = tensor((size_t)temb * 4), t_emb = tensor((size_t)temb * 4);
        int t_proj = tensor((size_t)u->tproj_total * 4);
        { Op o; o.kind = OP_SINUSOID; o.out = t_sin; o.N = c0; push(o); }
        { Op o; o.kind = OP_GEMV; o.x1 = t_sin; o.out = t_h1; o.N = temb; o.K = c0; o.w = W("time_embedding.linear_1.weight"); o.b = W("time_embedding.linear_1.bias"); push(o); }
        { Op o; o.kind = OP_GEMV; o.x1 = t_h1; o.out = t_emb; o.N = temb; o.K = temb; o.silu_in = 1; o.w = W("time_embedding.linear_2.weight"); o.b = W("time_embedding.linear_2.bias"); push(o); }
        { Op o; o.kind = OP_GEMV; o.x1 = t_emb; o.out = t_proj; o.N = (int)u->tproj_total; o.K = temb; o.silu_in = 1; o.w = W("tproj.weight"); o.b = W("tproj.bias"); push(o); }
        int rh = pl.lh, rw = pl.lw;
        int h;
        if (pl.rep > 1) { prefix_rep = pl.rep; UB /= pl.rep; }
        { Op o; o.kind = OP_CONV_IN; o.x1 = T_LATENTS; o.B = UB; o.Hin = rh; o.Win = rw; o.Cin = c.in_channels; o.N = c0;
          o.w = W("conv_in.weight"); o.b = W("conv_in.bias"); o.out = tensor((size_t)UB * rh * rw * c0 * 2); push(o); h = o.out; }
        const int h_skip = prefix_rep > 1 ? replicate(h, (size_t)UB * rh * rw * c0 * 2, prefix_rep) : h;
        pl.taps["conv_in"] = h_skip;
        int ch = c0;
        std::vector<int> skips{h_skip}, skip_ch{c0};
        for (int i = 0; i < nl; ++i) {
            const int co = c.block_out_channels[i];
            const std::string bp = "down_blocks." + std::to_string(i) + ".";
            wrapstack.push_back(Wrap{0, i, 0});
            for (int j = 0; j < c.layers_per_block; ++j) {
                wrapstack.push_back(Wrap{0, i, j});
                h = resnet(bp + "resnets." + std::to_string(j) + ".", h, ch, -1, 0, co, rh, rw, t_proj);
                ch = co;
                if (c.attn_levels[i]) h = transformer(bp + "attentions." + std::to_string(j) + ".", h, co, rh, rw);
                wrapstack.pop_back();
                skips.push_back(h); skip_ch.push_back(co);
            }
            if (i < nl - 1) {
                wrapstack.push_back(Wrap{0, i, c.layers_per_block});
                const std::string d = bp + "downsamplers.0.conv.";
                h = conv3(h, rh, rw, co, co, 2, 0, d + "weight", d + "bias", 0, -1, -1);
                wrapstack.pop_back();
                rh /= 2; rw /= 2;
                skips.push_back(h); skip_ch.push_back(co);
            }
            wrapstack.pop_back();
            pl.taps["down" + std::to_string(i)] = h;
        }
        wrapstack.push_back(Wrap{1, 0, 0});
        h = resnet("mid_block.resnets.0.", h, ch, -1, 0, ch, rh, rw, t_proj);
        h = transformer("mid_block.attentions.0.", h, ch, rh, rw);
        h = resnet("mid_block.resnets.1.", h, ch, -1, 0, ch, rh, rw, t_proj);
        wrapstack.pop_back();
        pl.taps["mid"] = h;
        const int nres = c.layers_per_block + 1;
        for (int i = 0; i < nl; ++i) {
            const int lev = nl - 1 - i, co = c.block_out_channels[lev], rb = nl - 1 - i;
            const std::string bp = "up_blocks." + std::to_string(i) + ".";
            wrapstack.push_back(Wrap{2, rb, 0});
            for (int j = 0; j < nres; ++j) {
                const int s = skips.back(), sc = skip_ch.back();
                skips.pop_back(); skip_ch.pop_back();
                const int rl = nres - 1 - j;
                wrapstack.push_back(Wrap{2, rb, rl});
                h = resnet(bp + "resnets." + std::to_string(j) + ".", h, ch, s, sc, co, rh, rw, t_proj);
                ch = co;
                if (c.attn_levels[lev]) h = transformer(bp + "attentions." + std::to_string(j) + ".", h, co, rh, rw);
                wrapstack.pop_back();
            }
            if (i < nl - 1) {
                wrapstack.push_back(Wrap{2, rb, 0});
                const std::string up = bp + "upsamplers.0.conv.";
                h = conv3(h, rh, rw, co, co, 1, 1, up + "weight", up + "bias", 0, -1, -1);
                wrapstack.pop_back();
                rh *= 2; rw *= 2;
            }
            wrapstack.pop_back();
            pl.taps["up" + std::to_string(i)] = h;
        }
        int g = gn(h, ch, -1, 0, rh * rw, "conv_norm_out.weight", "conv_norm_out.bias", c.norm_eps, 1);
        { Op o; o.kind = OP_CONV_OUT; o.x1 = g; o.out = T_EPS; o.B = UB; o.Hin = rh; o.Win = rw; o.Cin = ch; o.N = c.out_channels;
          o.w = W("conv_out.weight"); o.b = W("conv_out.bias"); push(o); }
    }
};

bool wrap_skipped(const Wrap& w, int branch) {
    const int cache_layer_id = branch % 3, cache_block_id = branch / 3;
    if (w.block_i > cache_block_id || w.type == 1) return true;
    if (w.block_i < cache_block_id) return false;
    return w.type == 0 ? w.layer_i >= cache_layer_id : w.layer_i > cache_layer_id;
}

void op_tensors(const Op& o, int ins[12], int& nin) {
    nin = 0;
    for (int t : {o.x1, o.x2, o.r, o.b2t, o.wt, o.s1, o.s2, o.lnrs, o.slab_t, o.slab_r, o.slab_b2t})
        if (t >= 0) ins[nin++] = t;
}

void fuse_deferred_reduce(sd_unet* u, Plan& pl) {
    if (getenv("SD_GN_SLAB") && atoi(getenv("SD_GN_SLAB")) == 0) return;
    const int nops = (int)pl.ops.size();
    auto skipped = [&](const Op& o) {
        if (pl.branch < 0) return false;
        for (int k = 0; k < o.nwrap; ++k)
            if (wrap_skipped(o.wraps[k], pl.branch)) return true;
        return false;
    };
    std::vector<int> producer(pl.tensors.size(), -1);
    for (int i = 0; i < nops; ++i)
        if (pl.ops[i].out >= 0) producer[pl.ops[i].out] = i;
    for (int g = 0; g < nops; ++g) {
        Op& G = pl.ops[g];
        if (G.kind != OP_GN || G.out_fp8 || G.x1 < 0 || !sd_groupnorm_slab_ok(G.B, G.HW, G.C1, G.C2, u->cfg.norm_num_groups)) continue;
        const int p = producer[G.x1];
        if (p < 0 || p >= g) continue;
        Op& P = pl.ops[p];
        if (P.kind != OP_CONV3 && !(P.kind == OP_GEMM && P.epi == 0)) continue;
        if (P.splitk <= 1 || P.splitk > 64 || P.aux < 0 || P.dt || P.out_fp8 || P.defer || P.subpix) continue;
        if (P.kind == OP_GEMM && (P.coff || P.ldc_o || P.hm || P.rs >= 0 || P.lnrs >= 0)) continue;
        if ((long)G.B * G.HW != P.M || G.C1 != P.N || skipped(P) != skipped(G)) continue;
        bool first_reader = true;
        for (int i = p + 1; i < g && first_reader; ++i) {
            int ins[12], nin;
            op_tensors(pl.ops[i], ins, nin);
            for (int k = 0; k < nin; ++k)
                if (ins[k] == P.out) first_reader = false;
        }
        if (!first_reader) continue;
        P.defer = 1;
        G.slab_t = P.aux; G.slab_k = P.splitk; G.slab_b = P.b; G.slab_r = P.r;
        G.slab_b2t = P.kind == OP_CONV3 ? P.b2t : -1; G.slab_b2idx = P.b2idx;
    }
}

void assign_memory(sd_unet* u, Plan& pl) {
    const int nops = (int)pl.ops.size();
    pl.skipped.assign(nops, 0);
    if (pl.branch >= 0) {
        for (int i = 0; i < nops; ++i)
            for (int k = 0; k < pl.ops[i].nwrap; ++k)
                if (wrap_skipped(pl.ops[i].wraps[k], pl.branch)) pl.skipped[i] = 1;
        std::vector<int> producer(pl.tensors.size(), -1);
        for (int i = 0; i < nops; ++i) {
            if (pl.ops[i].out >= 0) producer[pl.ops[i].out] = i;
            if (pl.ops[i].stats >= 0) producer[pl.ops[i].stats] = i;
            if (pl.ops[i].rs >= 0) producer[pl.ops[i].rs] = i;
        }
        for (int i = 0; i < nops; ++i) {
            if (pl.skipped[i]) continue;
            int ins[12], nin;
            op_tensors(pl.ops[i], ins, nin);
            for (int k = 0; k < nin; ++k) {
                const int p = producer[ins[k]];
                if (p >= 0 && pl.skipped[p]) pl.tensors[ins[k]].persistent = true;
            }
        }
    }
    if (u->debug_taps)
        for (auto& kv : pl.taps) pl.tensors[kv.second].persistent = true;
    for (int i = 0; i < nops; ++i) {
        const Op& o = pl.ops[i];
        int ins[12], nin;
        op_tensors(o, ins, nin);
        for (int k = 0; k < nin; ++k) pl.tensors[ins[k]].last = std::max(pl.tensors[ins[k]].last, i);
        for (int t : {o.out, o.aux, o.stats, o.rs})
            if (t >= 0) {
                if (pl.tensors[t].def < 0) pl.tensors[t].def = i;
                pl.tensors[t].last = std::max(pl.tensors[t].last, i);
            }
    }
    size_t off = 0;
    for (auto& t : pl.tensors)
        if (t.ctx) { t.off = off; off += t.bytes; }
    for (auto& t : pl.tensors)
        if (t.persistent && !t.ctx) { t.off = off; off += t.bytes; }
    const size_t arena0 = off;
    struct Live { size_t off, bytes; int last; };
    std::vector<Live> live;
    size_t high = arena0;
    std::vector<std::vector<int>> def_at(nops);
    for (int t = 0; t < (int)pl.tensors.size(); ++t)
        if (!pl.tensors[t].persistent && pl.tensors[t].def >= 0) def_at[pl.tensors[t].def].push_back(t);
    for (int i = 0; i < nops; ++i) {
        for (int t : def_at[i]) {
            std::sort(live.begin(), live.end(), [](const Live& a, const Live& b) { return a.off < b.off; });
            size_t cur = arena0;
            for (const Live& l : live) {
                if (l.off >= cur + pl.tensors[t].bytes) break;
                cur = std::max(cur, l.off + l.bytes);
            }
            pl.tensors[t].off = cur;
            live.push_back(Live{cur, pl.tensors[t].bytes, pl.tensors[t].last});
            high = std::max(high, cur + pl.tensors[t].bytes);
        }
        live.erase(std::remove_if(live.begin(), live.end(), [i](const Live& l) { return l.last <= i; }), live.end());
    }
    pl.total_bytes = high + 4096;
}

static int plan_rep(const sd_unet* u, int latent_batch, int unet_batch) {
    static const bool off = getenv("SD_CFG_DEDUP") && atoi(getenv("SD_CFG_DEDUP")) == 0;
    return (!off && u->kind == 0 && u->cfg.attn_levels[0] && latent_batch > 0 && unet_batch == 2 * latent_batch) ? 2 : 1;
}

static int check_latent_size(const sd_unet* u, int lh, int lw, const char* who) {
    if (u->kind == 1 || u->kind == 4) {
        SD_REQUIRE(lh >= 8 && lw >= 8 && lh <= 128 && lw <= 128 && lh % 8 == 0 && lw % 8 == 0,
                   "%s: latent %dx%d (the VAE %s takes sides that are multiples of 8 in [8, 128])", who, lh, lw,
                   u->kind == 1 ? "decoder" : "encoder");
    } else if (u->kind == 0) {
        const int d = 1 << (u->cfg.num_levels - 1);
        SD_REQUIRE(lh >= d && lw >= d && lh <= 256 && lw <= 256 && lh % d == 0 && lw % d == 0,
                   "%s: latent %dx%d (both sides must be multiples of %d, at most 256)", who, lh, lw, d);
    }
    return 0;
}

int get_plan(sd_unet* u, int UB, int branch, Plan** out, int rep = 1, int lh = -1, int lw = -1) {
    SD_REQUIRE(u && u->finalized, "unet: parameters not finalized");
    SD_REQUIRE(UB > 0 && UB <= 4096, "unet: bad batch %d", UB);
    SD_REQUIRE(branch < 3 * u->cfg.num_levels, "unet: cache_branch_id %d out of range", branch);
    if (branch < 0) branch = -1;
    if (lh < 0) lh = u->cfg.sample_size;
    if (lw < 0) lw = u->cfg.sample_size;
    auto key = std::make_tuple(UB, branch, rep, lh, lw);
    auto it = u->plans.find(key);
    if (it == u->plans.end()) {
        if (lh != u->cfg.sample_size || lw != u->cfg.sample_size)
            if (check_latent_size(u, lh, lw, "unet")) return -1;
        Plan pl;
        pl.UB = UB;
        pl.branch = branch;
        pl.rep = rep;
        pl.lh = lh;
        pl.lw = lw;
        Builder b{u, pl, UB, {}};
        b.build();
        SD_REQUIRE(b.error.empty(), "unet: cannot build the plan for batch %d (cache branch %d, latent %dx%d): %s", UB, branch, lh, lw,
                   b.error.c_str());
        fuse_deferred_reduce(u, pl);
        assign_memory(u, pl);
        if (u->kind == 3) {
            int*& d = u->prep_tabs[std::make_pair(lh, lw)];
            if (!d) {
                SD_CHECK_HIP(hipMalloc((void**)&d, pl.prep_tab.size() * sizeof(int)));
                SD_CHECK_HIP(hipMemcpy(d, pl.prep_tab.data(), pl.prep_tab.size() * sizeof(int), hipMemcpyHostToDevice));
            }
            pl.dtab = d;
            std::vector<int>().swap(pl.prep_tab);
        }
        it = u->plans.emplace(key, std::move(pl)).first;
    }
    *out = &it->second;
    return 0;
}

int run_op(sd_unet* u, const Plan& pl, const Op& o, char* ws, const float* latents, int latent_batch, float* eps_out,
           float timestep, hipStream_t stream) {
    auto T = [&](int id) -> char* { return id >= 0 ? ws + pl.tensors[id].off : nullptr; };
    const char* wb = u->dweights;
    switch (o.kind) {
        case OP_SINUSOID:
            if (u->cond_set) return sd_launch_timestep_sinusoid_row(timestep, u->dcond, (float*)T(o.out), o.N, stream);
            return sd_launch_timestep_sinusoid(timestep, (float*)T(o.out), o.N, stream);
        case OP_GEMV:
            return sd_launch_gemv((const float*)T(o.x1), (const bf16_t*)(wb + o.w), (const float*)(wb + o.b),
                                  (float*)T(o.out), o.N, o.K, o.silu_in, stream);
        case OP_CONV_IN:
            return sd_launch_conv_in(o.x1 >= 0 ? (const float*)T(o.x1) : latents, o.x1 >= 0 ? o.B : latent_batch,
                                     (const float*)(wb + o.w), (const float*)(wb + o.b), (bf16_t*)T(o.out), o.B, o.Hin,
                                     o.Win, o.Cin, o.N, stream);
        case OP_PQCONV:
            return sd_launch_pqconv(latents, (const float*)(wb + o.w), (const float*)(wb + o.b), (float*)T(o.out), o.B,
                                    o.HW, timestep , stream);
        case OP_SOFTMAX:
            if (o.N > 4096) return sd_launch_softmax_rows_long((bf16_t*)T(o.x1), o.M, o.N, o.scale, stream);
            return sd_launch_softmax_rows((bf16_t*)T(o.x1), o.M, o.N, o.scale, stream);
        case OP_GN: {
            GroupNormArgs a;
            a.x1 = (const bf16_t*)T(o.x1); a.C1 = o.C1; a.x2 = (const bf16_t*)T(o.x2); a.C2 = o.C2;
            a.gamma = (const float*)(wb + o.g); a.beta = (const float*)(wb + o.be);
            a.y = (bf16_t*)T(o.out); a.partial = (float*)T(o.aux);
            a.B = o.B; a.HW = o.HW; a.groups = u->cfg.norm_num_groups; a.nsplit = o.nsplit; a.eps = o.eps; a.silu = o.silu;
            a.out_fp8 = o.out_fp8; a.Cpad = o.Cpad; a.oscale = o.os;
            a.stats1 = (const float*)T(o.s1); a.stats2 = (const float*)T(o.s2);
            if (o.slab_t >= 0) {
                a.slab = (const float*)T(o.slab_t); a.splitk = o.slab_k; a.x1w = (bf16_t*)T(o.x1);
                a.sbias = o.slab_b != NOFF ? (const float*)(wb + o.slab_b) : nullptr;
                a.sbias2 = o.slab_b2t >= 0 ? (const float*)T(o.slab_b2t) + o.slab_b2idx : nullptr;
                a.sR = (const bf16_t*)T(o.slab_r); a.sldr = o.C1;
            }
            return sd_launch_groupnorm(a, stream);
        }
        case OP_CONV3: {
            GemmArgs a;
            a.X = (const bf16_t*)T(o.x1); a.W = (const bf16_t*)(wb + o.w); a.bias = (const float*)(wb + o.b);
            a.bias2 = o.b2t >= 0 ? (const float*)T(o.b2t) + o.b2idx : nullptr;
            a.R = (const bf16_t*)T(o.r); a.ldr = o.N; a.C = (bf16_t*)T(o.out); a.ldc = o.N;
            a.M = o.M; a.N = o.N; a.K = o.K; a.K1 = o.K;
            a.Hin = o.Hin; a.Win = o.Win; a.Cin = o.Cin; a.Hout = o.Hout; a.Wout = o.Wout; a.stride = o.stride; a.up = o.up;
            a.zero_page = g_zero_page; a.splitk = o.splitk; a.slab = (float*)T(o.aux); a.defer_reduce = o.defer;
            if (o.dt) { a.dt = 1; a.wscale = (const float*)(wb + o.wsc); a.xscale_inv = 1.0f / o.xs; }
            a.stats = (float*)T(o.stats);
            a.asym = o.asym;
            if (o.subpix) { a.subpix = 1; a.up = 0; a.w_batch_stride = (long)o.N * 4 * o.Cin; }
            return sd_launch_conv3x3(a, stream);
        }
        case OP_GEMM: {
            GemmArgs a;
            a.X = o.wx != NOFF ? (const bf16_t*)(wb + o.wx) : (const bf16_t*)T(o.x1) + o.xoff;
            a.ldx = o.ldx_o ? o.ldx_o : o.K1; a.X2 = (const bf16_t*)T(o.x2); a.ldx2 = o.K - o.K1; a.K1 = o.K1;
            a.W = o.wt >= 0 ? (const bf16_t*)T(o.wt) + o.woff_el : (const bf16_t*)(wb + o.w); a.ldw = o.ldw_o;
            a.bias = o.b != NOFF ? (const float*)(wb + o.b) : nullptr;
            a.R = (const bf16_t*)T(o.r); a.ldr = o.N; a.C = (bf16_t*)T(o.out) + o.coff;
            a.ldc = o.ldc_o ? o.ldc_o : (o.epi == 1 ? o.N / 2 : o.N);
            a.M = o.M; a.N = o.N; a.K = o.K; a.zero_page = g_zero_page; a.splitk = o.splitk; a.slab = (float*)T(o.aux);
            a.defer_reduce = o.defer;
            a.w_batch_stride = o.wbs; a.rows_per_batch = o.rpb; a.sm_valid = o.sm_valid;
            if (o.dt) { a.dt = 1; a.wscale = (const float*)(wb + o.wsc); a.xscale_inv = 1.0f / o.xs; }
            if (o.out_fp8) { a.out_fp8 = 1; a.oscale = o.os; a.ldc = o.Cpad; }
            a.stats = (float*)T(o.stats);
            a.rowstats = (float*)T(o.rs);
            if (o.hm) { a.hm_C = o.N / 3; a.hm_tok = o.HW; a.ldc = a.hm_C; a.KV = (bf16_t*)T(o.out) + (long)o.M * a.hm_C; }
            if (o.lnrs >= 0) { a.ln_rs = (const float*)T(o.lnrs); a.ln_np = o.lnnp; a.ln_c1 = (const float*)(wb + o.c1); a.ln_eps = 1e-5f; }
            if (o.lnrs >= 0 && o.s1 >= 0) { a.ln_c1 = (const float*)T(o.s1); a.bias = (const float*)T(o.s2); a.ln_per_sample = 1; }
            return sd_launch_gemm(a, o.epi, stream);
        }
        case OP_LN:
            if (o.out_fp8)
                return sd_launch_layernorm_fp8((const bf16_t*)T(o.x1), (const float*)(wb + o.g), (const float*)(wb + o.be),
                                               T(o.out), o.M, o.N, o.Cpad, o.eps, o.os, stream);
            return sd_launch_layernorm((const bf16_t*)T(o.x1), (const float*)(wb + o.g), (const float*)(wb + o.be),
                                       (bf16_t*)T(o.out), o.M, o.N, o.eps, stream);
        case OP_ATTN: {
            AttnArgs a;
            a.Q = (const bf16_t*)T(o.x1) + o.qoff; a.ldq = o.ldq;
            a.K = (const bf16_t*)T(o.x2) + o.koff; a.ldk = o.ldk;
            a.V = (const bf16_t*)T(o.x2) + o.voff; a.ldv = o.ldv;
            a.O = (bf16_t*)T(o.out); a.ldo = o.ldo;
            a.B = o.B; a.heads = o.heads; a.Nq = o.Nq; a.Nk = o.Nk; a.D = o.D;
            a.scale = 1.0f / sqrtf((float)o.D);
            a.q_prescaled = o.qps;
            a.consts = g_zero_page;
            a.kv_head_major = o.hm;
            return sd_launch_attention(a, stream);
        }
        case OP_XATTN: {
            XattnArgs a;
            a.X = (const bf16_t*)T(o.x1); a.R = (const bf16_t*)T(o.r); a.Y = (bf16_t*)T(o.out);
            a.At = (const bf16_t*)T(o.wt); a.Bw = (const bf16_t*)T(o.x2); a.bias = (const float*)(wb + o.b);
            a.M = o.M; a.C = o.N; a.rows_per_sample = o.rpb; a.L = o.sm_valid;
            a.rowstats = (float*)T(o.rs);
            if (o.lnrs >= 0) {
                a.ln_rs = (const float*)T(o.lnrs); a.ln_np = o.lnnp; a.ln_rows = o.ldx_o; a.ln_c2 = (const float*)T(o.s1); a.ln_eps = 1e-5f;
            }
            return sd_launch_xattn_fused(a, stream);
        }
        case OP_REPLICATE:
            return sd_launch_replicate(T(o.x1), T(o.out), (long)o.M * 16, o.N, stream);
        case OP_CLIP_EMBED:
            return sd_launch_clip_embed((const int*)latents, (const bf16_t*)(wb + o.w), (const bf16_t*)(wb + o.g),
                                        (bf16_t*)T(o.out), o.M, o.Nk, o.N, u->clip.vocab_size, stream);
        case OP_CLIP_ATTN:
            return sd_launch_clip_attention((const bf16_t*)T(o.x1), (bf16_t*)T(o.out), o.B, o.Nq, o.N, o.heads, stream);
        case OP_QGELU:
            return sd_launch_quick_gelu((bf16_t*)T(o.x1), (long)o.M * o.N, stream);
        case OP_VIT_PREP:
            return sd_launch_clip_preprocess((const unsigned char*)latents, o.B, pl.geom, pl.dtab, (unsigned char*)T(o.aux),
                                             (bf16_t*)T(o.out), o.Cin, o.K, nullptr, stream);
        case OP_VIT_EMBED:
            return sd_launch_vit_embed((const bf16_t*)T(o.x1), (const float*)(wb + o.b), (const bf16_t*)(wb + o.g),
                                       (bf16_t*)T(o.out), o.B, o.Nq, o.N, stream);
        case OP_VIT_ATTN:
            return sd_launch_vit_attention((const bf16_t*)T(o.x1), (bf16_t*)T(o.out), o.B, o.Nq, o.N, o.heads, stream);
        case OP_POOL:
            return sd_launch_pool_rows((const bf16_t*)T(o.x1), o.pool_by_ids ? (const int*)latents : nullptr, o.B, o.Nq, o.N, u->eos_id,
                                       (bf16_t*)T(o.out), stream);
        case OP_TO_F32:
            return sd_launch_bf16_to_f32((const bf16_t*)T(o.x1), eps_out, (long)o.M * o.N, stream);
        case OP_CONV_IN_IMG:
            return sd_launch_conv_in_image(latents, (const float*)(wb + o.w), (const float*)(wb + o.b), (bf16_t*)T(o.out), o.B,
                                           o.Hin, o.Win, o.N, stream);
        case OP_ENC_OUT:
            return sd_launch_vae_enc_out((const bf16_t*)T(o.x1), (const bf16_t*)(wb + o.w), (const float*)(wb + o.b),
                                         (const float*)(wb + o.g), (const float*)(wb + o.be), eps_out, o.B, o.Hin, o.Win, o.Cin,
                                         stream);
        case OP_CONV_OUT:
            return sd_launch_conv_out((const bf16_t*)T(o.x1), (const bf16_t*)(wb + o.w), (const float*)(wb + o.b), eps_out,
// ... 727 lines not shown

extern "C" int sd_sched_step(void* stream, const float* eps, int cfg, float guidance, const float* x, const float* m1,
                             const float* m2, const float* m3, const float* noise, float* prev, float* y2, float* m_out,
                             const float coef[10], long long n) {
    SD_REQUIRE(coef, "sched_step: null coefficients");
    StepCoef c{coef[0], coef[1], coef[2], coef[3], coef[4], coef[5], coef[6], coef[7], coef[8], coef[9]};
    return sd_launch_sched_step(eps, cfg, guidance, x, m1, m2, m3, noise, prev, y2, m_out, c, (long)n, (hipStream_t)stream);
}

extern "C" int sd_cfg_rescale_factors(void* stream, const float* eps, int batch, long long n_per_sample, float guidance,
                                      float rescale, float* k_out) {
    return sd_launch_cfg_rescale_factors(eps, batch, (long)n_per_sample, guidance, rescale, k_out, (hipStream_t)stream);
}

extern "C" int sd_sched_step_rescaled(void* stream, const float* eps, int cfg, float guidance, const float* x,
                                      const float* m1, const float* m2, const float* m3, const float* noise, float* prev,
                                      float* y2, float* m_out, const float coef[10], long long n, const float* k,
                                      long long n_per_sample) {
    SD_REQUIRE(coef, "sched_step_rescaled: null coefficients");
    StepCoef c{coef[0], coef[1], coef[2], coef[3], coef[4], coef[5], coef[6], coef[7], coef[8], coef[9]};
    return sd_launch_sched_step_rescaled(eps, cfg, guidance, x, m1, m2, m3, noise, prev, y2, m_out, c, k, (long)n_per_sample,
                                         (long)n, (hipStream_t)stream);
}

extern "C" int sd_op_gemm(void* stream, const void* X, long long ldx, const void* X2, long long ldx2, int K1,
                          const void* W, const float* bias, const float* bias2, const void* R, long long ldr, void* C,
                          long long ldc, int M, int N, int K, int epi) {
    if (ensure_zero_page()) return -2;
    GemmArgs a;
    a.X = (const bf16_t*)X; a.ldx = ldx; a.X2 = (const bf16_t*)X2; a.ldx2 = ldx2; a.K1 = K1;
    a.W = (const bf16_t*)W; a.bias = bias; a.bias2 = bias2; a.R = (const bf16_t*)R; a.ldr = ldr;
    a.C = (bf16_t*)C; a.ldc = ldc; a.M = M; a.N = N; a.K = K; a.zero_page = g_zero_page;
    a.splitk = epi ? 1 : sd_gemm_splitk(M, N, K);
    if (a.splitk > 1) {
        a.slab = (float*)op_scratch((size_t)a.splitk * M * N * 4);
        SD_REQUIRE(a.slab, "sd_op_gemm: cannot allocate split-K scratch");
    }
    return sd_launch_gemm(a, epi, (hipStream_t)stream);
}

extern "C" int sd_op_gemm_batched(void* stream, const void* X, long long ldx, const void* W, long long w_batch_stride,
                                  int rows_per_batch, const float* bias, const void* R, long long ldr, void* C,
                                  long long ldc, int M, int N, int K, int epi, int sm_valid) {
    if (ensure_zero_page()) return -2;
    SD_REQUIRE(epi == 0 || epi == 2, "sd_op_gemm_batched: epi %d (0 = std, 2 = softmax over 80-column groups)", epi);
    GemmArgs a;
    a.X = (const bf16_t*)X; a.ldx = ldx; a.K1 = K; a.W = (const bf16_t*)W; a.bias = bias; a.R = (const bf16_t*)R; a.ldr = ldr;
    a.C = (bf16_t*)C; a.ldc = ldc; a.M = M; a.N = N; a.K = K; a.zero_page = g_zero_page;
    a.w_batch_stride = w_batch_stride; a.rows_per_batch = rows_per_batch; a.sm_valid = sm_valid; a.splitk = 1;
    return sd_launch_gemm(a, epi, (hipStream_t)stream);
}

extern "C" int sd_op_gemm_batched_softmax_ln(void* stream, const void* X, long long ldx, const void* W, long long w_batch_stride,
                                             int rows_per_batch, void* C, long long ldc, int M, int N, int K, int sm_valid,
                                             const float* rowstats, int parts, const float* c1, const float* c2, float eps) {
    if (ensure_zero_page()) return -2;
    SD_REQUIRE(rowstats && c1 && c2, "sd_op_gemm_batched_softmax_ln: null operand");
    GemmArgs a;
    a.X = (const bf16_t*)X; a.ldx = ldx; a.K1 = K; a.W = (const bf16_t*)W; a.bias = c2;
    a.C = (bf16_t*)C; a.ldc = ldc; a.M = M; a.N = N; a.K = K; a.zero_page = g_zero_page;
    a.w_batch_stride = w_batch_stride; a.rows_per_batch = rows_per_batch; a.sm_valid = sm_valid; a.splitk = 1;
    a.ln_rs = rowstats; a.ln_np = parts; a.ln_c1 = c1; a.ln_eps = eps; a.ln_per_sample = 1;
    return sd_launch_gemm(a, 2, (hipStream_t)stream);
}

extern "C" int sd_op_conv3x3(void* stream, const void* X, const void* W, const float* bias, const float* bias2,
                             const void* R, void* Y, int B, int Hin, int Win, int Cin, int Cout, int stride, int upsample) {
    if (ensure_zero_page()) return -2;
    SD_REQUIRE(stride == 1 || stride == 2, "conv3x3: stride %d", stride);
    GemmArgs a;
    a.X = (const bf16_t*)X; a.W = (const bf16_t*)W; a.bias = bias; a.bias2 = bias2; a.R = (const bf16_t*)R; a.ldr = Cout;
    a.C = (bf16_t*)Y; a.ldc = Cout;
    a.Hin = Hin; a.Win = Win; a.Cin = Cin; a.stride = stride; a.up = upsample ? 1 : 0;
    a.Hout = ((Hin << a.up) + 2 - 3) / stride + 1; a.Wout = ((Win << a.up) + 2 - 3) / stride + 1;
    a.M = B * a.Hout * a.Wout; a.N = Cout; a.K = 9 * Cin; a.K1 = a.K; a.zero_page = g_zero_page;
    a.splitk = sd_conv3x3_splitk(a.M, a.N, Cin, Hin, Win, stride, a.up);
    if (a.splitk > 1) {
        a.slab = (float*)op_scratch((size_t)a.splitk * a.M * a.N * 4);
        SD_REQUIRE(a.slab, "sd_op_conv3x3: cannot allocate split-K scratch");
    }
    return sd_launch_conv3x3(a, (hipStream_t)stream);
}

extern "C" int sd_op_conv3x3_down_asym(void* stream, const void* X, const void* W, const float* bias, void* Y, int B, int Hin,
                                       int Win, int Cin, int Cout) {
    if (ensure_zero_page()) return -2;
    SD_REQUIRE(X && W && Y && B > 0 && Hin > 0 && Win > 0 && Hin % 2 == 0 && Win % 2 == 0,
               "conv3x3_down_asym: even input sides (%dx%d)", Hin, Win);
    GemmArgs a;
    a.X = (const bf16_t*)X; a.W = (const bf16_t*)W; a.bias = bias; a.C = (bf16_t*)Y; a.ldc = Cout;
    a.Hin = Hin; a.Win = Win; a.Cin = Cin; a.stride = 2; a.up = 0; a.asym = 1;
    a.Hout = Hin / 2; a.Wout = Win / 2;
    a.M = B * a.Hout * a.Wout; a.N = Cout; a.K = 9 * Cin; a.K1 = a.K; a.zero_page = g_zero_page;
    a.splitk = sd_conv3x3_splitk(a.M, a.N, Cin, Hin, Win, 2, 0);
    if (a.splitk > 1) {
        a.slab = (float*)op_scratch((size_t)a.splitk * a.M * a.N * 4);
        SD_REQUIRE(a.slab, "sd_op_conv3x3_down_asym: cannot allocate split-K scratch");
    }
    return sd_launch_conv3x3(a, (hipStream_t)stream);
}

extern "C" int sd_op_conv3x3_kernel(int M, int N, int Cin, int Hin, int Win, int stride, int upsample, int dtype) {
    SD_REQUIRE(M > 0 && N > 0 && Cin > 0 && Hin > 0 && Win > 0 && (stride == 1 || stride == 2) && upsample >= 0 && upsample <= 2 &&
                   (dtype == 0 || dtype == 1), "conv3x3_kernel: bad arguments");
    GemmArgs a;
    a.M = M; a.N = N; a.Cin = Cin; a.Hin = Hin; a.Win = Win; a.stride = stride; a.dt = dtype;
    if (upsample == 2) {
        a.subpix = 1; a.up = 0; a.K = 4 * Cin; a.ldw = a.K; a.Hout = 2 * Hin; a.Wout = 2 * Win;
        a.w_batch_stride = (long)N * a.K; a.splitk = 1;
        return sd_conv_halo_subpix_applicable(a) ? 2 : 0;
    }
    a.up = upsample; a.K = 9 * Cin; a.ldw = a.K;
    a.Hout = ((Hin << a.up) + 2 - 3) / stride + 1; a.Wout = ((Win << a.up) + 2 - 3) / stride + 1;
    return sd_conv_halo_mode(a) != 0 ? 1 : 0;
}

extern "C" int sd_op_softmax_rows(void* stream, void* S, long long rows, int cols, float scale) {
    if (cols > 4096) return sd_launch_softmax_rows_long((bf16_t*)S, rows, cols, scale, (hipStream_t)stream);
    return sd_launch_softmax_rows((bf16_t*)S, rows, cols, scale, (hipStream_t)stream);
}

extern "C" int sd_op_conv3x3_ablate(void* stream, const void* X, const void* W, void* Y, int B, int Hin, int Win, int Cin, int Cout,
                                    int ablate) {
    if (ensure_zero_page()) return -2;
    const int abl = ablate & ~256;
    SD_REQUIRE(abl == 0 || abl == 8 || (!(ablate & 256) && (abl == 1 || abl == 2 || abl == 4)), "conv3x3_ablate: mode %d", ablate);
    GemmArgs a;
    a.X = (const bf16_t*)X; a.W = (const bf16_t*)W; a.C = (bf16_t*)Y; a.ldc = Cout; a.ldr = Cout;
    a.Hin = Hin; a.Win = Win; a.Cin = Cin; a.stride = 1; a.up = 0; a.Hout = Hin; a.Wout = Win;
    a.M = B * Hin * Win; a.N = Cout; a.K = 9 * Cin; a.K1 = a.K; a.zero_page = g_zero_page; a.splitk = 1; a.tune = ablate;
    SD_REQUIRE(Cin % 64 == 0 && Cout % 4 == 0 && sd_conv_halo_applicable(a), "conv3x3_ablate: not a halo-kernel shape");
    return sd_launch_conv3x3_halo(a, (hipStream_t)stream);
}

extern "C" int sd_op_conv3x3_upsample_subpixel(void* stream, const void* X, const void* W4, const float* bias, void* Y, int B,
                                               int Hin, int Win, int Cin, int Cout) {
    if (ensure_zero_page()) return -2;
    GemmArgs a;
    a.X = (const bf16_t*)X; a.W = (const bf16_t*)W4; a.bias = bias; a.C = (bf16_t*)Y; a.ldc = Cout;
    a.Hin = Hin; a.Win = Win; a.Cin = Cin; a.stride = 1; a.up = 0; a.Hout = 2 * Hin; a.Wout = 2 * Win;
    a.M = 4 * B * Hin * Win; a.N = Cout; a.K = 4 * Cin; a.K1 = a.K; a.zero_page = g_zero_page; a.splitk = 1;
    a.subpix = 1; a.w_batch_stride = (long)Cout * 4 * Cin;
    return sd_launch_conv3x3(a, (hipStream_t)stream);
}

extern "C" int sd_op_conv3x3_upsample_subpixel_groupnorm(void* stream, const void* X, const void* W4, const float* bias, void* Y,
                                                         int B, int Hin, int Win, int Cin, int Cout, const float* gamma,
                                                         const float* beta, void* Yn, int groups, float eps, int silu) {
    if (ensure_zero_page()) return -2;
    const int HW = 4 * Hin * Win;
    SD_REQUIRE((Hin * Win) % 128 == 0 && !sd_groupnorm_uses_small(B, HW, Cout, 0, groups),
               "sd_op_conv3x3_upsample_subpixel_groupnorm: %dx%d -> x2, %d channels: no producer statistics at this size", Hin, Win, Cout);
    const size_t stats_bytes = (size_t)B * (HW / 64) * Cout * 2 * 4;
    char* scratch = (char*)op_scratch(stats_bytes + sd_groupnorm_scratch_bytes(B, HW, groups));
    SD_REQUIRE(scratch, "sd_op_conv3x3_upsample_subpixel_groupnorm: cannot allocate scratch");
    GemmArgs a;
    a.X = (const bf16_t*)X; a.W = (const bf16_t*)W4; a.bias = bias; a.C = (bf16_t*)Y; a.ldc = Cout;
    a.Hin = Hin; a.Win = Win; a.Cin = Cin; a.stride = 1; a.up = 0; a.Hout = 2 * Hin; a.Wout = 2 * Win;
    a.M = 4 * B * Hin * Win; a.N = Cout; a.K = 4 * Cin; a.K1 = a.K; a.zero_page = g_zero_page; a.splitk = 1;
    a.subpix = 1; a.w_batch_stride = (long)Cout * 4 * Cin;
    a.stats = (float*)scratch;
    if (int rc = sd_launch_conv3x3(a, (hipStream_t)stream)) return rc;
    GroupNormArgs g;
    g.x1 = (const bf16_t*)Y; g.C1 = Cout; g.gamma = gamma; g.beta = beta; g.y = (bf16_t*)Yn; g.B = B; g.HW = HW;
    g.groups = groups; g.eps = eps; g.silu = silu; g.nsplit = sd_groupnorm_nsplit(B, HW);
    g.partial = (float*)(scratch + stats_bytes);
// ... 303 lines not shown
```

Baseline: 11.29 images/s.

## Fold ResNet 1x1 shortcut GEMM into the conv2 halo kernel as extra K-phase

When a ResNet block changes channel count, the 1x1 shortcut projection is now accumulated inside the conv2 3x3 halo kernel as an additional K phase, reading the block input (optionally two concatenated segments) and the shortcut weights. The biases are pre-summed at load time. This removes a separate GEMM launch and the write-then-read of the shortcut residual tensor, at the cost of more K work per conv2 tile and a new kernel instantiation. It is on by default and can be disabled with SD_SHORTCUT_FUSE=0. New C entry points expose the fused op.

```diff
diff --git a/include/sd_hip.h b/include/sd_hip.h
--- a/include/sd_hip.h
+++ b/include/sd_hip.h
@@ -170,6 +170,11 @@
                                   const float* rowstats, int parts, const float* c1, const float* c2, float eps);
 int sd_op_conv3x3(void* stream, const void* X, const void* W, const float* bias, const float* bias2, const void* R,
                   void* Y, int B, int Hin, int Win, int Cin, int Cout, int stride, int upsample);
+int sd_op_conv3x3_shortcut(void* stream, const void* X, const void* W, const float* bias, const void* Xs1, int Cs1,
+                           const void* Xs2, int Cs2, const void* Wsc, void* Y, int B, int H, int Wd, int Cin, int Cout);
+int sd_op_conv3x3_shortcut_groupnorm(void* stream, const void* X, const void* W, const float* bias, const void* Xs1, int Cs1,
+                                     const void* Xs2, int Cs2, const void* Wsc, void* Y, int B, int H, int Wd, int Cin,
+                                     int Cout, const float* gamma, const float* beta, void* Yn, int groups, float eps, int silu);
 int sd_op_conv3x3_down_asym(void* stream, const void* X, const void* W, const float* bias, void* Y, int B, int Hin, int Win,
                             int Cin, int Cout);
 int sd_op_conv3x3_kernel(int M, int N, int Cin, int Hin, int Win, int stride, int upsample, int dtype);
diff --git a/sonicdiffusionbayeslab_amd/_lib.py b/sonicdiffusionbayeslab_amd/_lib.py
--- a/sonicdiffusionbayeslab_amd/_lib.py
+++ b/sonicdiffusionbayeslab_amd/_lib.py
@@ -119,6 +119,9 @@
     "sd_op_gemm_batched": (_i, [_vp, _vp, _ll, _vp, _ll, _i, _vp, _vp, _ll, _vp, _ll, _i, _i, _i, _i, _i]),
     "sd_op_gemm_batched_softmax_ln": (_i, [_vp, _vp, _ll, _vp, _ll, _i, _vp, _ll, _i, _i, _i, _i, _vp, _i, _vp, _vp, _f]),
     "sd_op_conv3x3": (_i, [_vp, _vp, _vp, _vp, _vp, _vp, _vp, _i, _i, _i, _i, _i, _i, _i]),
+    "sd_op_conv3x3_shortcut": (_i, [_vp, _vp, _vp, _vp, _vp, _i, _vp, _i, _vp, _vp, _i, _i, _i, _i, _i]),
+    "sd_op_conv3x3_shortcut_groupnorm": (_i, [_vp, _vp, _vp, _vp, _vp, _i, _vp, _i, _vp, _vp, _i, _i, _i, _i, _i,
+                                              _vp, _vp, _vp, _i, _f, _i]),
     "sd_op_conv3x3_down_asym": (_i, [_vp, _vp, _vp, _vp, _vp, _i, _i, _i, _i, _i]),
     "sd_op_conv3x3_ablate": (_i, [_vp, _vp, _vp, _vp, _i, _i, _i, _i, _i, _i]),
     "sd_op_conv3x3_upsample_subpixel": (_i, [_vp, _vp, _vp, _vp, _vp, _i, _i, _i, _i, _i]),
diff --git a/sonicdiffusionbayeslab_amd/csrc/conv_halo.hip b/sonicdiffusionbayeslab_amd/csrc/conv_halo.hip
--- a/sonicdiffusionbayeslab_amd/csrc/conv_halo.hip
+++ b/sonicdiffusionbayeslab_amd/csrc/conv_halo.hip
@@ -25,9 +25,10 @@
 
 __device__ __forceinline__ int swz_of(int row, int dt) { return dt ? (((row >> 1) & 1) | (row & 4)) : (row & 7); }
 
-template <int DT, int DIAG = 0, int NWV = 8, int SUB = 0, int GEN = 0>
+template <int DT, int DIAG = 0, int NWV = 8, int SUB = 0, int GEN = 0, int SC = 0>
 __global__ __launch_bounds__(NWV * 64, NWV == 8 ? 2 : 1) void conv_halo_kernel(const GemmArgs p) {
     static_assert(NWV == 8 || (NWV == 4 && DT == 0), "4-wave layout: bf16 only");
+    static_assert(!SC || (DT == 0 && DIAG == 0 && NWV == 8 && SUB == 0), "shortcut phase: bf16, 8 waves, 9 taps");
     static_assert(!SUB || (DT == 0 && DIAG == 0 && NWV == 8), "sub-pixel upsampler: bf16, 8 waves");
     static_assert(!GEN || (SUB == 0 && DIAG == 0 && NWV == 8), "geometry mode: 9 taps, 8 waves");
     constexpr int NTAP = SUB ? 4 : 9;
@@ -202,6 +203,11 @@
     const int wfrag = (wn * WTN + lrow) * 128;
     const int wswz0 = DT ? ((2 * lq) ^ swz_of(lane, 1)) << 4 : (lq ^ (lane & 7)) << 4;
 
+    const int sc_gch = ((lane & 7) ^ (lane >> 3)) << 4;
+    const int scp1 = SC ? p.Csc1 * 2 : 0, scp2 = SC ? p.Csc2 * 2 : 0, scpw = SC ? (int)p.ldwsc * 2 : 0;
+    const int vXs1 = (lane >> 3) * scp1 + sc_gch, vXs2 = (lane >> 3) * scp2 + sc_gch, vWs = (lane >> 3) * scpw + sc_gch;
+    const int scfrag = (wm * WTM + lrow) * 128 + ((lq ^ (lane & 7)) << 4);
+
     auto frag_addr = [&](int f, int tp) -> int {
         const int hp = hbase[f] + (((hrc[f] >> 16) + (tp / 3 - 1)) >> up) * PW + (((hrc[f] & 0xffff) + (tp % 3 - 1)) >> up);
         return hp * 128 + (DT ? (((2 * lq) ^ swz_of(hp, 1)) << 4) : ((lq ^ (hp & 7)) << 4));
@@ -388,6 +394,63 @@
         }
         if (CARRY) mfmas(xf1, wf1);
 
+        if (SC) {
+            const int nsc = (p.Csc1 + p.Csc2) >> 6, nsc1 = p.Csc1 >> 6;
+            const int t_begin = (int)((long)nsc * split / p.splitk), t_end = (int)((long)nsc * (split + 1) / p.splitk);
+            if (t_begin < t_end) {
+                const unsigned rows = (unsigned)(GEN ? min(mend, p.M) : p.M);
+                auto stage_sc = [&](int t, char* xb, char* wb) {
+                    const bool seg1 = t < nsc1;
+                    const int pitch = seg1 ? scp1 : scp2;
+                    const __amdgpu_buffer_rsrc_t rx = __builtin_amdgcn_make_buffer_rsrc((void*)(seg1 ? p.Xs1 : p.Xs2), 0,
+                                                                                        (int)(rows * (unsigned)pitch), 0x00020000);
+                    const int vx = seg1 ? vXs1 : vXs2;
+                    const int so = (m0 + wave * 8) * pitch + (seg1 ? t : t - nsc1) * 128;
+#pragma unroll
+                    for (int i = 0; i < BM / 64; ++i)
+                        __builtin_amdgcn_raw_ptr_buffer_load_lds(rx, LDS_PTR(xb + (wave + 8 * i) * 1024), 16, vx, so + i * 64 * pitch, 0, 0);
+                    const __amdgpu_buffer_rsrc_t rw = __builtin_amdgcn_make_buffer_rsrc((void*)p.Wsc, 0, (int)((unsigned)p.N * (unsigned)scpw), 0x00020000);
+#pragma unroll
+                    for (int i = 0; i < WPW; ++i) {
+                        const int pc = wpiece(i);
+                        __builtin_amdgcn_raw_ptr_buffer_load_lds(rw, LDS_PTR(wb + pc * 1024), 16, vWs, (n0 + pc * 8) * scpw + t * 128, 0, 0);
+                    }
+                };
+                char* const xlast = hsel ? Hb0 : Hb1;
+                char* const xprev = hsel ? Hb1 : Hb0;
+                char* const wlast = Wb + (wst == 0 ? 2 : wst - 1) * WBYTES;
+                char* const wprev = Wb + wst * WBYTES;
+                wait_vmcnt<0>();
+                __builtin_amdgcn_s_barrier();
+                asm volatile("" ::: "memory");
+                {
+                    const bool e0 = ((t_end - 1 - t_begin) & 1) == 0;
+                    stage_sc(t_begin, e0 ? xlast : xprev, e0 ? wlast : wprev);
+                }
+                for (int t = t_begin; t < t_end; ++t) {
+                    const bool e = ((t_end - 1 - t) & 1) == 0;
+                    const char* xcur = e ? xlast : xprev;
+                    const char* wcur = e ? wlast : wprev;
+                    wait_vmcnt<0>();
+                    __builtin_amdgcn_s_barrier();
+                    asm volatile("" ::: "memory");
+#pragma unroll
+                    for (int f = 0; f < TM; ++f) xf0[f] = *(const bf16x8*)(xcur + scfrag + f * 2048);
+#pragma unroll
+                    for (int a = 0; a < TN; ++a) wf0[a] = *(const bf16x8*)(wcur + wfrag + a * 2048 + wswz0);
+                    __builtin_amdgcn_sched_barrier(0);
+                    if (t + 1 < t_end) stage_sc(t + 1, e ? xprev : xlast, e ? wprev : wlast);
+                    __builtin_amdgcn_sched_barrier(0);
+#pragma unroll
+                    for (int f = 0; f < TM; ++f) xf1[f] = *(const bf16x8*)(xcur + ((scfrag + f * 2048) ^ 64));
+#pragma unroll
+                    for (int a = 0; a < TN; ++a) wf1[a] = *(const bf16x8*)(wcur + wfrag + a * 2048 + (wswz0 ^ 64));
+                    mfmas(xf0, wf0);
+                    mfmas(xf1, wf1);
+                }
+            }
+        }
+
         const int em0 = m0, en0 = n0, esplit = split, ephase = phase;
         const int elim = GEN ? mend : Mrows;
         auto crow = [&](int m) -> long {
@@ -405,7 +468,7 @@
             }
         }
         if (p.splitk == 1) {
-            if (p.R) {
+            if (SC == 0 && p.R) {
                 u32x2 rr[TN][TM];
 #pragma unroll
                 for (int a = 0; a < TN; ++a) {
@@ -429,7 +492,7 @@
                 for (int a = 0; a < TN; ++a) {
                     const int n = min(en0 + wn * WTN + a * 16 + lq * 4, p.N - 4);
                     f32x4 bv = *(const f32x4*)(p.bias + n);
-                    if (p.bias2) bv += *(const f32x4*)(p.bias2 + n);
+                    if (SC == 0 && p.bias2) bv += *(const f32x4*)(p.bias2 + n);
 #pragma unroll
                     for (int b = 0; b < TM; ++b) acc[a][b] += bv;
                 }
@@ -557,6 +620,16 @@
     if ((long)a.M * a.Cin * 2 >= (1l << 32) || (long)a.N * ldw * 2 >= (1l << 32)) return false;
     if (a.dt == 1 && a.Cin % 128) return false;
     return true;
+}
+
+bool sd_conv_halo_shortcut_applicable(const GemmArgs& a) {
+    if (a.dt != 0 || a.subpix || a.up || a.stride != 1 || a.R != nullptr || a.bias2 != nullptr || a.tune != 0) return false;
+    if (!sd_conv_halo_applicable(a)) return false;
+    if (a.Csc1 < 64 || a.Csc1 % 64 || a.Csc2 < 0 || a.Csc2 % 64) return false;
+    const long ldw = a.ldwsc ? a.ldwsc : a.Csc1 + a.Csc2;
+    if (ldw < a.Csc1 + a.Csc2 || (ldw & 7)) return false;
+    const long big = 1l << 32;
+    return ((long)a.M + BM) * std::max(a.Csc1, a.Csc2) * 2 < big && ((long)a.N + BN) * ldw * 2 < big;
 }
 
 bool sd_conv_halo_subpix_applicable(const GemmArgs& a) {
@@ -619,11 +692,18 @@
     }
     const int slices = a.Cin / (a.dt ? 128 : 64);
     SD_REQUIRE(a.splitk <= slices, "conv3x3 halo: splitk %d exceeds the %d channel slices", a.splitk, slices);
+    if (a.Wsc) {
+        SD_REQUIRE(a.Xs1 && (a.Xs2 || a.Csc2 == 0) && sd_conv_halo_shortcut_applicable(a0),
+                   "conv3x3 halo: the 1x1 shortcut (%d + %d channels) cannot ride on this conv", a.Csc1, a.Csc2);
+        if (a.ldwsc == 0) a.ldwsc = a.Csc1 + a.Csc2;
+        if (a.Csc2 == 0) a.Xs2 = a.Xs1;
+    }
     if (!pow2_applicable(a0)) return launch_halo_gen(a, stream);
     static bool attr_set = false;
     if (!attr_set) {
         SD_CHECK_HIP(hipFuncSetAttribute((const void*)conv_halo_kernel<0>, hipFuncAttributeMaxDynamicSharedMemorySize, SMEM));
         SD_CHECK_HIP(hipFuncSetAttribute((const void*)conv_halo_kernel<1>, hipFuncAttributeMaxDynamicSharedMemorySize, SMEM));
+        SD_CHECK_HIP(hipFuncSetAttribute((const void*)conv_halo_kernel<0, 0, 8, 0, 0, 1>, hipFuncAttributeMaxDynamicSharedMemorySize, SMEM));
 #ifdef SD_ABLATE
         SD_CHECK_HIP(hipFuncSetAttribute((const void*)conv_halo_kernel<0, 1>, hipFuncAttributeMaxDynamicSharedMemorySize, SMEM));
         SD_CHECK_HIP(hipFuncSetAttribute((const void*)conv_halo_kernel<0, 3>, hipFuncAttributeMaxDynamicSharedMemorySize, SMEM));
@@ -636,6 +716,13 @@
     }
     int grid = a.tiles_m * a.tiles_n * a.splitk;
     if (grid > 256) grid = 256;
+    if (a.Wsc) {
+        a.tune = 0;
+        hipLaunchKernelGGL((conv_halo_kernel<0, 0, 8, 0, 0, 1>), dim3(grid), dim3(512), SMEM, stream, a);
+        if (a.splitk > 1 && !a.defer_reduce) sd_launch_splitk_reduce(a, stream);
+        SD_CHECK_HIP(hipGetLastError());
+        return 0;
+    }
 #ifdef SD_ABLATE
     const int tune = a0.tune;
     a.tune = tune;
@@ -670,11 +757,13 @@
     if (!attr_set) {
         SD_CHECK_HIP(hipFuncSetAttribute((const void*)conv_halo_kernel<0, 0, 8, 0, 1>, hipFuncAttributeMaxDynamicSharedMemorySize, SMEM));
         SD_CHECK_HIP(hipFuncSetAttribute((const void*)conv_halo_kernel<1, 0, 8, 0, 1>, hipFuncAttributeMaxDynamicSharedMemorySize, SMEM));
+        SD_CHECK_HIP(hipFuncSetAttribute((const void*)conv_halo_kernel<0, 0, 8, 0, 1, 1>, hipFuncAttributeMaxDynamicSharedMemorySize, SMEM));
         attr_set = true;
     }
     int grid = a.tiles_m * a.tiles_n * a.splitk;
     if (grid > 256) grid = 256;
-    if (a.dt) hipLaunchKernelGGL((conv_halo_kernel<1, 0, 8, 0, 1>), dim3(grid), dim3(512), SMEM, stream, a);
+    if (a.Wsc) hipLaunchKernelGGL((conv_halo_kernel<0, 0, 8, 0, 1, 1>), dim3(grid), dim3(512), SMEM, stream, a);
+    else if (a.dt) hipLaunchKernelGGL((conv_halo_kernel<1, 0, 8, 0, 1>), dim3(grid), dim3(512), SMEM, stream, a);
     else hipLaunchKernelGGL((conv_halo_kernel<0, 0, 8, 0, 1>), dim3(grid), dim3(512), SMEM, stream, a);
     if (a.splitk > 1 && !a.defer_reduce) sd_launch_splitk_reduce(a, stream);
     SD_CHECK_HIP(hipGetLastError());
diff --git a/sonicdiffusionbayeslab_amd/csrc/gemm_conv.hip b/sonicdiffusionbayeslab_amd/csrc/gemm_conv.hip
--- a/sonicdiffusionbayeslab_amd/csrc/gemm_conv.hip
+++ b/sonicdiffusionbayeslab_amd/csrc/gemm_conv.hip
@@ -780,6 +780,8 @@
                "conv3x3: output size %dx%d inconsistent with input %dx%d stride %d up %d", a.Hout, a.Wout,
                a.Hin, a.Win, a.stride, a.up);
     SD_REQUIRE(a.M % (a.Hout * a.Wout) == 0, "conv3x3: M not a multiple of Hout*Wout");
+    SD_REQUIRE(!a.Wsc || sd_conv_halo_shortcut_applicable(a), "conv3x3: the 1x1 shortcut (%d + %d channels) cannot ride on this conv",
+               a.Csc1, a.Csc2);
     if (sd_conv_halo_applicable(a)) return sd_launch_conv3x3_halo(a, stream);
     if (a.dt == 1) return launch<128, 160, 2, 2, 2, AMODE_CONV, EPI_STD, 1>(a, stream);
     if (big_tile_ok(a.M, a.N, 160)) return launch<256, 160, 4, 2, 3, AMODE_CONV, EPI_STD>(a, stream);
diff --git a/sonicdiffusionbayeslab_amd/csrc/kernels.h b/sonicdiffusionbayeslab_amd/csrc/kernels.h
--- a/sonicdiffusionbayeslab_amd/csrc/kernels.h
+++ b/sonicdiffusionbayeslab_amd/csrc/kernels.h
@@ -44,6 +44,11 @@
     float xscale_inv = 1.0f;
     int out_fp8 = 0;
     float oscale = 1.0f;
+    const bf16_t* Xs1 = nullptr;
+    const bf16_t* Xs2 = nullptr;
+    const bf16_t* Wsc = nullptr;
+    long ldwsc = 0;
+    int Csc1 = 0, Csc2 = 0;
 };
 
 int sd_gemm_tile_rows(int M, int N, int K = 0);
@@ -58,6 +63,7 @@
 int sd_conv3x3_splitk(int M, int N, int Cin, int Hin, int Win, int stride, int up, int dt = 0);
 bool sd_conv_halo_subpix_applicable(const GemmArgs& a);
 int sd_launch_conv3x3_halo(const GemmArgs& a, hipStream_t stream);
+bool sd_conv_halo_shortcut_applicable(const GemmArgs& a);
 
 struct GroupNormArgs {
     const bf16_t* x1 = nullptr; int C1 = 0;
diff --git a/sonicdiffusionbayeslab_amd/csrc/unet.hip b/sonicdiffusionbayeslab_amd/csrc/unet.hip
--- a/sonicdiffusionbayeslab_amd/csrc/unet.hip
+++ b/sonicdiffusionbayeslab_amd/csrc/unet.hip
@@ -112,6 +112,8 @@
     size_t c1 = NOFF;
     size_t wsc = NOFF;
     float xs = 1.f, os = 1.f;
+    int scx1 = -1, scx2 = -1, scc1 = 0, scc2 = 0;
+    size_t scw = NOFF;
     int nwrap = 0;
     Wrap wraps[3];
 };
@@ -730,7 +732,14 @@
         f32(p + "conv2.bias");
         if (u->fp8) { conv3_fp8(p + "conv1.weight", cout, cin); conv3_fp8(p + "conv2.weight", cout, cout); }
         else { conv3(p + "conv1.weight", cout, cin); conv3(p + "conv2.weight", cout, cout); }
-        if (cin != cout) { bf16_same(p + "conv_shortcut.weight"); f32(p + "conv_shortcut.bias"); }
+        if (cin != cout) {
+            bf16_same(p + "conv_shortcut.weight"); f32(p + "conv_shortcut.bias");
+            const auto& b2 = P(p + "conv2.bias");
+            const auto& bs = P(p + "conv_shortcut.bias");
+            const size_t off = alloc(p + "conv2.bias+shortcut", b2.size() * 4);
+            float* o = (float*)(u->hblob.data() + off);
+            for (size_t i = 0; i < b2.size(); ++i) o[i] = b2[i] + bs[i];
+        }
     }
     void transformer(const std::string& p, int c) {
         f32(p + "norm.weight"); f32(p + "norm.bias");
@@ -1170,6 +1179,7 @@
         push(o);
         return o.out;
     }
+    bool shortcut_fuse = !(getenv("SD_SHORTCUT_FUSE") && atoi(getenv("SD_SHORTCUT_FUSE")) == 0);
     int resnet(const std::string& p, int x1, int c1, int x2, int c2, int cout, int rh, int rw, int tproj_t) {
         const int hw = rh * rw, cin = c1 + c2, M = UB * hw;
         const bool fq = u->fp8;
@@ -1177,7 +1187,19 @@
         int t2 = conv3(t1, rh, rw, cin, cout, 1, 0, p + "conv1.weight", p + "conv1.bias", u->tproj_off.at(p), tproj_t, -1, fq);
         int t3 = gn(t2, cout, -1, 0, hw, p + "norm2.weight", p + "norm2.bias", u->cfg.norm_eps, 1, fq);
         int sc = x1;
-        if (cin != cout) sc = gemm(x1, c1, x2, c2, M, cout, p + "conv_shortcut.weight", p + "conv_shortcut.bias", -1, 0);
+        if (cin != cout) {
+            GemmArgs g;
+            g.M = M; g.N = cout; g.Cin = cout; g.K = 9 * cout; g.ldw = g.K; g.Hin = g.Hout = rh; g.Win = g.Wout = rw;
+            g.Csc1 = c1; g.Csc2 = x2 >= 0 ? c2 : 0;
+            if (shortcut_fuse && !fq && u->kind == 0 && u->woff.count(p + "conv2.bias+shortcut") && sd_conv_halo_shortcut_applicable(g)) {
+                const int out = conv3(t3, rh, rw, cout, cout, 1, 0, p + "conv2.weight", p + "conv2.bias+shortcut", 0, -1, -1, fq);
+                Op& o = pl.ops.back();
+                o.scx1 = x1; o.scc1 = c1; o.scx2 = x2; o.scc2 = g.Csc2; o.scw = W(p + "conv_shortcut.weight");
+                o.Kalg += cin;
+                return out;
+            }
+            sc = gemm(x1, c1, x2, c2, M, cout, p + "conv_shortcut.weight", p + "conv_shortcut.bias", -1, 0);
+        }
         return conv3(t3, rh, rw, cout, cout, 1, 0, p + "conv2.weight", p + "conv2.bias", 0, -1, sc, fq);
     }
     int n_transformers = 0;
@@ -1558,9 +1580,9 @@
     return w.type == 0 ? w.layer_i >= cache_layer_id : w.layer_i > cache_layer_id;
 }
 
-void op_tensors(const Op& o, int ins[12], int& nin) {
+void op_tensors(const Op& o, int ins[16], int& nin) {
     nin = 0;
-    for (int t : {o.x1, o.x2, o.r, o.b2t, o.wt, o.s1, o.s2, o.lnrs, o.slab_t, o.slab_r, o.slab_b2t})
+    for (int t : {o.x1, o.x2, o.r, o.b2t, o.wt, o.s1, o.s2, o.lnrs, o.slab_t, o.slab_r, o.slab_b2t, o.scx1, o.scx2})
         if (t >= 0) ins[nin++] = t;
 }
 
@@ -1588,7 +1610,7 @@
         if ((long)G.B * G.HW != P.M || G.C1 != P.N || skipped(P) != skipped(G)) continue;
         bool first_reader = true;
         for (int i = p + 1; i < g && first_reader; ++i) {
-            int ins[12], nin;
+            int ins[16], nin;
             op_tensors(pl.ops[i], ins, nin);
             for (int k = 0; k < nin; ++k)
                 if (ins[k] == P.out) first_reader = false;
@@ -1615,7 +1637,7 @@
         }
         for (int i = 0; i < nops; ++i) {
             if (pl.skipped[i]) continue;
-            int ins[12], nin;
+            int ins[16], nin;
             op_tensors(pl.ops[i], ins, nin);
             for (int k = 0; k < nin; ++k) {
                 const int p = producer[ins[k]];
@@ -1627,7 +1649,7 @@
         for (auto& kv : pl.taps) pl.tensors[kv.second].persistent = true;
     for (int i = 0; i < nops; ++i) {
         const Op& o = pl.ops[i];
-        int ins[12], nin;
+        int ins[16], nin;
         op_tensors(o, ins, nin);
         for (int k = 0; k < nin; ++k) pl.tensors[ins[k]].last = std::max(pl.tensors[ins[k]].last, i);
         for (int t : {o.out, o.aux, o.stats, o.rs})
@@ -1771,6 +1793,10 @@
             a.stats = (float*)T(o.stats);
             a.asym = o.asym;
             if (o.subpix) { a.subpix = 1; a.up = 0; a.w_batch_stride = (long)o.N * 4 * o.Cin; }
+            if (o.scw != NOFF) {
+                a.Xs1 = (const bf16_t*)T(o.scx1); a.Csc1 = o.scc1; a.Xs2 = (const bf16_t*)T(o.scx2); a.Csc2 = o.scc2;
+                a.Wsc = (const bf16_t*)(wb + o.scw); a.ldwsc = o.scc1 + o.scc2;
+            }
             return sd_launch_conv3x3(a, stream);
         }
         case OP_GEMM: {
@@ -2664,6 +2690,58 @@
     return sd_launch_conv3x3(a, (hipStream_t)stream);
 }
 
+static int conv3x3_shortcut_args(GemmArgs& a, const void* X, const void* W, const float* bias, const void* Xs1, int Cs1,
+                                 const void* Xs2, int Cs2, const void* Wsc, void* Y, int B, int H, int Wd, int Cin, int Cout) {
+    SD_REQUIRE(X && W && Xs1 && Wsc && Y && B > 0 && H > 0 && Wd > 0 && Cin > 0 && Cout > 0 && Cs1 > 0 && Cs2 >= 0 && (Xs2 || Cs2 == 0),
+               "conv3x3_shortcut: bad arguments");
+    a.X = (const bf16_t*)X; a.W = (const bf16_t*)W; a.bias = bias; a.C = (bf16_t*)Y; a.ldc = Cout;
+    a.Hin = a.Hout = H; a.Win = a.Wout = Wd; a.Cin = Cin; a.stride = 1; a.up = 0;
+    a.M = B * H * Wd; a.N = Cout; a.K = 9 * Cin; a.K1 = a.K; a.zero_page = g_zero_page;
+    a.Xs1 = (const bf16_t*)Xs1; a.Csc1 = Cs1; a.Xs2 = (const bf16_t*)Xs2; a.Csc2 = Cs2; a.Wsc = (const bf16_t*)Wsc; a.ldwsc = Cs1 + Cs2;
+    SD_REQUIRE(Cin % 64 == 0 && sd_conv_halo_shortcut_applicable(a),
+               "conv3x3_shortcut: %dx%d, %d -> %d channels with a %d + %d channel shortcut is not a shape the halo kernel folds", H, Wd,
+               Cin, Cout, Cs1, Cs2);
+    return 0;
+}
+
+extern "C" int sd_op_conv3x3_shortcut(void* stream, const void* X, const void* W, const float* bias, const void* Xs1, int Cs1,
+                                      const void* Xs2, int Cs2, const void* Wsc, void* Y, int B, int H, int Wd, int Cin, int Cout) {
+    if (ensure_zero_page()) return -2;
+    GemmArgs a;
+    if (int rc = conv3x3_shortcut_args(a, X, W, bias, Xs1, Cs1, Xs2, Cs2, Wsc, Y, B, H, Wd, Cin, Cout)) return rc;
+    a.splitk = sd_conv3x3_splitk(a.M, a.N, Cin, H, Wd, 1, 0);
+    if (a.splitk > 1) {
+        a.slab = (float*)op_scratch((size_t)a.splitk * a.M * a.N * 4);
+        SD_REQUIRE(a.slab, "sd_op_conv3x3_shortcut: cannot allocate split-K scratch");
+    }
+    return sd_launch_conv3x3(a, (hipStream_t)stream);
+}
+
+extern "C" int sd_op_conv3x3_shortcut_groupnorm(void* stream, const void* X, const void* W, const float* bias, const void* Xs1,
+                                                int Cs1, const void* Xs2, int Cs2, const void* Wsc, void* Y, int B, int H, int Wd,
+                                                int Cin, int Cout, const float* gamma, const float* beta, void* Yn, int groups,
+                                                float eps, int silu) {
+    if (ensure_zero_page()) return -2;
+    const int HW = H * Wd;
+    SD_REQUIRE(HW % 64 == 0 && !sd_groupnorm_uses_small(B, HW, Cout, 0, groups),
+               "sd_op_conv3x3_shortcut_groupnorm: %dx%d pixels per sample: producer statistics come in 64-pixel blocks", H, Wd);
+    GemmArgs a;
+    if (int rc = conv3x3_shortcut_args(a, X, W, bias, Xs1, Cs1, Xs2, Cs2, Wsc, Y, B, H, Wd, Cin, Cout)) return rc;
+    const size_t stats_bytes = (size_t)B * (HW / 64) * Cout * 2 * 4;
+    char* scratch = (char*)op_scratch(stats_bytes + sd_groupnorm_scratch_bytes(B, HW, groups));
+    SD_REQUIRE(scratch, "sd_op_conv3x3_shortcut_groupnorm: cannot allocate scratch");
+    a.splitk = 1;
+    a.stats = (float*)scratch;
+    SD_REQUIRE(sd_conv_halo_mode(a) == 1, "sd_op_conv3x3_shortcut_groupnorm: the geometry mode delivers no block statistics");
+    if (int rc = sd_launch_conv3x3(a, (hipStream_t)stream)) return rc;
+    GroupNormArgs g;
+    g.x1 = (const bf16_t*)Y; g.C1 = Cout; g.gamma = gamma; g.beta = beta; g.y = (bf16_t*)Yn; g.B = B; g.HW = HW;
+    g.groups = groups; g.eps = eps; g.silu = silu; g.nsplit = sd_groupnorm_nsplit(B, HW);
+    g.partial = (float*)(scratch + stats_bytes);
+    g.stats1 = (const float*)scratch;
+    return sd_launch_groupnorm(g, (hipStream_t)stream);
+}
+
 extern "C" int sd_op_conv3x3_down_asym(void* stream, const void* X, const void* W, const float* bias, void* Y, int B, int Hin,
                                        int Win, int Cin, int Cout) {
     if (ensure_zero_page()) return -2;
```

After: 11.40 images/s, median of 6. +1.0%, better.
